# teofum/platinum

Hardware: AMD Instinct MI355X
Metric: Msamples/s (paths x spp x bounces / s) at 1920x1080, 8 bounces (higher is better)
Workload: dtype f32; 1 GPU; C3 1.04M-triangle instanced sphere field, 1920x1080; width=1920, height=1080, max_bounces=8, samples_in_flight=128, spp_per_gpu=1792, spp_total=1792, integrator=MIS+NEE, flags=MultiscatterGGX, triangles=1036300, call_pattern=render(spp_per_step) per step, batches=14, nonfinite_policy=zero (a NaN/inf sample counts as black; parity default is propagate), parallelism=sample-sharded x1, one process per GPU + RCCL all-reduce

## Files before the change

include/ptamd.h:

```cpp
#ifndef PTAMD_H
#define PTAMD_H

#include <stdint.h>

#ifdef __cplusplus
extern "C" {
#endif

#define PT_ABI_VERSION 5u


enum { PT_STATUS_BLOCKED = 0, PT_STATUS_READY = 1, PT_STATUS_BUSY = 4, PT_STATUS_DONE = 8 };
enum { PT_INTEGRATOR_SIMPLE = 0, PT_INTEGRATOR_MIS = 1 };
enum { PT_FLAG_NONE = 0, PT_FLAG_MULTISCATTER_GGX = 1 << 0, PT_FLAG_GMON = 1 << 1 };
enum { PT_NONFINITE_PROPAGATE = 0, PT_NONFINITE_ZERO = 1 };
enum {
  PT_MATERIAL_THIN_DIELECTRIC = 1 << 0,
  PT_MATERIAL_USE_ALPHA = 1 << 1,
  PT_MATERIAL_EMISSIVE = 1 << 2,
  PT_MATERIAL_ANISOTROPIC = 1 << 3
};

typedef enum pt_error {
  PT_OK = 0,
// ... 219 lines not shown
  float agx_offset[3], agx_slope[3], agx_power[3], agx_saturation;
  float khr_compression_start, khr_desaturation;
  float flim_pre_exposure, flim_pre_formation_filter[3], flim_pre_formation_filter_strength;
  float flim_extended_gamut_scale[3], flim_extended_gamut_rotation[3], flim_extended_gamut_mul[3];
  float flim_sigmoid_log2_min, flim_sigmoid_log2_max, flim_sigmoid_toe[2], flim_sigmoid_shoulder[2];
  float flim_negative_exposure, flim_negative_density, flim_print_backlight[3], flim_print_exposure, flim_print_density;
  float flim_black_point;
  uint32_t flim_auto_black_point;
  float flim_post_formation_filter[3], flim_post_formation_filter_strength, flim_midtone_saturation;
  float shadow_color[3], midtone_color[3], highlight_color[3];
  float shadow_offset, midtone_offset, highlight_offset;
  pt_colorspace output_space;
} pt_tonemap_options;

void pt_default_post_options(pt_post_options* o);
void pt_default_tonemap_options(pt_tonemap_options* o);
int pt_set_post_options(pt_renderer* r, const pt_post_options* o);
int pt_set_tonemap_options(pt_renderer* r, const pt_tonemap_options* o);
int pt_read_render_target(pt_renderer* r, uint8_t* rgba8_out);
int pt_present_render_target(pt_renderer* r, void** device_rgba8_out, void** stream_out);

int pt_read_accumulator(pt_renderer* r, float* rgba_out);
void* pt_accumulator_device_ptr(pt_renderer* r);


typedef struct pt_denoise_options {
  uint32_t enabled;
  uint32_t iterations;
  float sigma_luminance, sigma_normal, sigma_depth;
  uint32_t apply_to_target;
} pt_denoise_options;
enum { PT_AOV_ALBEDO = 0, PT_AOV_NORMAL = 1, PT_AOV_MOMENTS = 2 };
void pt_default_denoise_options(pt_denoise_options* o);
int pt_set_denoise_options(pt_renderer* r, const pt_denoise_options* o);
int pt_read_aov(pt_renderer* r, uint32_t aov, float* rgba_out);
int pt_read_denoised(pt_renderer* r, float* rgba_out);

typedef struct pt_despeckle_options {
  uint32_t enabled;
  float threshold;
} pt_despeckle_options;
void pt_default_despeckle_options(pt_despeckle_options* o);
int pt_set_despeckle_options(pt_renderer* r, const pt_despeckle_options* o);

typedef struct pt_exposure_options {
  uint32_t enabled;
  float target_log2;
  float low_fraction;
  float high_fraction;
  float min_ev, max_ev;
  float smoothing;
} pt_exposure_options;
void pt_default_exposure_options(pt_exposure_options* o);
int pt_set_exposure_options(pt_renderer* r, const pt_exposure_options* o);
int pt_reset_exposure(pt_renderer* r);

typedef struct pt_exposure_meter {
  uint32_t bins[256];
  uint32_t below, above, nonfinite, metered;
  uint32_t kept;  uint32_t _pad;  uint64_t weighted;
  float mean_log2, target_ev, ev, gain;
} pt_exposure_meter;
int pt_read_exposure_meter(pt_renderer* r, pt_exposure_meter* out);
int pt_debug_exposure(pt_renderer* r, const float* rgba, uint32_t width, uint32_t height, const uint32_t* rect,
                      const pt_exposure_options* options, pt_exposure_meter* out, float* scaled_out);

typedef struct pt_adaptive_options {
  uint32_t enabled;
  float threshold;
  uint32_t min_spp;
  uint32_t interval;
} pt_adaptive_options;
void pt_default_adaptive_options(pt_adaptive_options* o);
int pt_set_adaptive_options(pt_renderer* r, const pt_adaptive_options* o);
int pt_read_sample_counts(pt_renderer* r, uint32_t* out);

typedef struct pt_render_region {
  uint32_t enabled;
  uint32_t x0, y0, x1, y1;
} pt_render_region;
void pt_default_render_region(pt_render_region* o);
int pt_set_render_region(pt_renderer* r, const pt_render_region* o);
int pt_region_tiles(uint32_t width, uint32_t height, const pt_render_region* o, uint32_t* tiles_out, uint32_t capacity, uint32_t* count);

const char* pt_last_error(void);


int pt_get_constants(const pt_renderer* r, pt_constants* out);
int pt_get_env_alias(const pt_renderer* r, pt_alias_entry* out, uint64_t capacity, uint64_t* count);
int pt_get_lights(const pt_renderer* r, pt_area_light* out, uint32_t capacity, uint32_t* count);

typedef struct pt_hit_record {
  float t, u, v;
  int32_t instance;
  int32_t primitive;
} pt_hit_record;
int pt_trace_primary(pt_renderer* r, uint32_t sample_idx, pt_hit_record* out );

int pt_debug_sample(pt_renderer* r, uint32_t sample_idx, float* radiance_out, int32_t* hits_out);

typedef struct pt_stats {
  uint64_t triangles;
  uint64_t bvh_nodes;
  uint32_t bvh_max_depth;
  uint32_t samples_in_flight;
  double upload_ms;
  double bvh_build_ms;
  uint64_t closest_rays;
  uint64_t shadow_rays;
  uint64_t shaded_hits;
  uint64_t paths;
  uint64_t nonfinite_samples;
  double ms_raygen, ms_closest, ms_shade, ms_shadow, ms_accumulate;
  uint64_t launches_closest, launches_shadow;
  double nodes_per_closest_ray, tris_per_closest_ray;
  double nodes_per_shadow_ray, tris_per_shadow_ray;
  uint32_t accel_two_level;
  uint32_t batches;
  uint64_t leaf_slots;
} pt_stats;
int pt_get_stats(pt_renderer* r, pt_stats* out);
int pt_set_profiling(pt_renderer* r, int enabled);
int pt_measure_traversal(pt_renderer* r, uint32_t sample_idx);

#ifdef __cplusplus
}
#endif
#endif
```

platinum_amd/abi.py:

```python
import ctypes as C
import os

PT_ABI_VERSION = 5

STATUS_BLOCKED, STATUS_READY, STATUS_BUSY, STATUS_DONE = 0, 1, 4, 8
INTEGRATOR_SIMPLE, INTEGRATOR_MIS = 0, 1
FLAG_NONE, FLAG_MULTISCATTER_GGX, FLAG_GMON = 0, 1, 2
MATERIAL_THIN_DIELECTRIC, MATERIAL_USE_ALPHA, MATERIAL_EMISSIVE, MATERIAL_ANISOTROPIC = 1, 2, 4, 8
NONFINITE_PROPAGATE, NONFINITE_ZERO = 0, 1
ACCEL_AUTO, ACCEL_ONE_BVH, ACCEL_TWO_LEVEL = 0, 1, 2


class Float3(C.Structure):
    _fields_ = [("x", C.c_float), ("y", C.c_float), ("z", C.c_float), ("_pad", C.c_float)]


class VertexData(C.Structure):
    _fields_ = [("normal", Float3), ("tangent", C.c_float * 4), ("texCoords", C.c_float * 2), ("_pad", C.c_float * 2)]


class MaterialGPU(C.Structure):
    _fields_ = [
        ("baseColor", C.c_float * 4), ("emission", Float3), ("emissionStrength", C.c_float),
        ("roughness", C.c_float), ("metallic", C.c_float), ("transmission", C.c_float), ("ior", C.c_float),
# ... 81 lines not shown


class CreateInfo(C.Structure):
    _fields_ = [
        ("abi_version", C.c_uint32), ("device_ordinal", C.c_int32), ("lut_blob", C.c_void_p),
        ("lut_blob_size", C.c_uint64), ("lut_path", C.c_char_p),
        ("device_ordinals", C.POINTER(C.c_int32)), ("device_count", C.c_uint32),
    ]


class RenderParams(C.Structure):
    _fields_ = [
        ("width", C.c_uint32), ("height", C.c_uint32), ("spp", C.c_uint32), ("gmon_buckets", C.c_uint32),
        ("flags", C.c_int32), ("integrator", C.c_uint32), ("working_space", Colorspace),
        ("max_bounces", C.c_uint32), ("first_sample", C.c_uint32), ("samples_in_flight", C.c_uint32),
        ("nonfinite_policy", C.c_uint32), ("external_accumulator", C.c_void_p), ("stream", C.c_void_p),
        ("accel_structure", C.c_uint32), ("_reserved", C.c_uint32),
    ]


class QueuePlan(C.Structure):
    _fields_ = [("samples_in_flight", C.c_uint32), ("tiles_per_seg", C.c_uint32), ("nseg", C.c_uint32), ("seg_cap", C.c_uint32),
                ("capacity", C.c_uint64), ("lbuf_entries", C.c_uint64)]


class GmonOptions(C.Structure):
    _fields_ = [("cap", C.c_float)]


class PostOptions(C.Structure):
    _fields_ = [(n, C.c_float) for n in (
        "exposure", "ca_amount", "ca_green_shift", "contrast", "saturation", "blacks", "shadows", "highlights", "whites",
        "vig_amount", "vig_midpoint", "vig_feather", "vig_power", "vig_roundness")]


class TonemapOptions(C.Structure):
    _fields_ = [
        ("tonemapper", C.c_uint32), ("agx_offset", C.c_float * 3), ("agx_slope", C.c_float * 3), ("agx_power", C.c_float * 3),
        ("agx_saturation", C.c_float), ("khr_compression_start", C.c_float), ("khr_desaturation", C.c_float),
        ("flim_pre_exposure", C.c_float), ("flim_pre_formation_filter", C.c_float * 3), ("flim_pre_formation_filter_strength", C.c_float),
        ("flim_extended_gamut_scale", C.c_float * 3), ("flim_extended_gamut_rotation", C.c_float * 3), ("flim_extended_gamut_mul", C.c_float * 3),
        ("flim_sigmoid_log2_min", C.c_float), ("flim_sigmoid_log2_max", C.c_float), ("flim_sigmoid_toe", C.c_float * 2),
        ("flim_sigmoid_shoulder", C.c_float * 2), ("flim_negative_exposure", C.c_float), ("flim_negative_density", C.c_float),
        ("flim_print_backlight", C.c_float * 3), ("flim_print_exposure", C.c_float), ("flim_print_density", C.c_float),
        ("flim_black_point", C.c_float), ("flim_auto_black_point", C.c_uint32), ("flim_post_formation_filter", C.c_float * 3),
        ("flim_post_formation_filter_strength", C.c_float), ("flim_midtone_saturation", C.c_float),
        ("shadow_color", C.c_float * 3), ("midtone_color", C.c_float * 3), ("highlight_color", C.c_float * 3),
        ("shadow_offset", C.c_float), ("midtone_offset", C.c_float), ("highlight_offset", C.c_float), ("output_space", Colorspace),
    ]


TONEMAP_NONE, TONEMAP_AGX, TONEMAP_KHRONOS_PBR, TONEMAP_FLIM = 0, 1, 2, 3


class DenoiseOptions(C.Structure):
    _fields_ = [("enabled", C.c_uint32), ("iterations", C.c_uint32), ("sigma_luminance", C.c_float), ("sigma_normal", C.c_float),
                ("sigma_depth", C.c_float), ("apply_to_target", C.c_uint32)]


AOV_ALBEDO, AOV_NORMAL, AOV_MOMENTS = 0, 1, 2


class DespeckleOptions(C.Structure):
    _fields_ = [("enabled", C.c_uint32), ("threshold", C.c_float)]


class ExposureOptions(C.Structure):
    _fields_ = [("enabled", C.c_uint32), ("target_log2", C.c_float), ("low_fraction", C.c_float), ("high_fraction", C.c_float),
                ("min_ev", C.c_float), ("max_ev", C.c_float), ("smoothing", C.c_float)]


class ExposureMeter(C.Structure):
    _fields_ = [("bins", C.c_uint32 * 256), ("below", C.c_uint32), ("above", C.c_uint32), ("nonfinite", C.c_uint32), ("metered", C.c_uint32),
                ("kept", C.c_uint32), ("_pad", C.c_uint32), ("weighted", C.c_uint64),
                ("mean_log2", C.c_float), ("target_ev", C.c_float), ("ev", C.c_float), ("gain", C.c_float)]


class AdaptiveOptions(C.Structure):
    _fields_ = [("enabled", C.c_uint32), ("threshold", C.c_float), ("min_spp", C.c_uint32), ("interval", C.c_uint32)]


class RenderRegion(C.Structure):
    _fields_ = [("enabled", C.c_uint32), ("x0", C.c_uint32), ("y0", C.c_uint32), ("x1", C.c_uint32), ("y1", C.c_uint32)]


class HitRecord(C.Structure):
    _fields_ = [("t", C.c_float), ("u", C.c_float), ("v", C.c_float), ("instance", C.c_int32), ("primitive", C.c_int32)]


class Stats(C.Structure):
    _fields_ = [
        ("triangles", C.c_uint64), ("bvh_nodes", C.c_uint64), ("bvh_max_depth", C.c_uint32),
        ("samples_in_flight", C.c_uint32), ("upload_ms", C.c_double), ("bvh_build_ms", C.c_double),
        ("closest_rays", C.c_uint64), ("shadow_rays", C.c_uint64), ("shaded_hits", C.c_uint64), ("paths", C.c_uint64),
        ("nonfinite_samples", C.c_uint64), ("ms_raygen", C.c_double), ("ms_closest", C.c_double), ("ms_shade", C.c_double), ("ms_shadow", C.c_double),
        ("ms_accumulate", C.c_double), ("launches_closest", C.c_uint64), ("launches_shadow", C.c_uint64),
        ("nodes_per_closest_ray", C.c_double), ("tris_per_closest_ray", C.c_double),
        ("nodes_per_shadow_ray", C.c_double), ("tris_per_shadow_ray", C.c_double),
        ("accel_two_level", C.c_uint32), ("batches", C.c_uint32), ("leaf_slots", C.c_uint64),
    ]


class RuntimeInfo(C.Structure):
    _fields_ = [
        ("hip_runtime_path", C.c_char * 512), ("hsa_runtime_path", C.c_char * 512), ("rccl_path", C.c_char * 512),
        ("hip_runtimes_mapped", C.c_uint32), ("hsa_runtimes_mapped", C.c_uint32), ("rccl_mapped", C.c_uint32),
        ("hip_runtime_version", C.c_int32), ("all_mapped", C.c_char * 2048),
    ]


assert C.sizeof(Float3) == 16 and C.sizeof(VertexData) == 48 and C.sizeof(MaterialGPU) == 96
assert C.sizeof(Instance) == 64 and C.sizeof(CameraData) == 80 and C.sizeof(Constants) == 176
assert C.sizeof(AreaLight) == 48

SYMBOLS = [
    ("pt_create", C.c_int, [C.POINTER(CreateInfo), C.POINTER(C.c_void_p)]),
    ("pt_group_partition", C.c_int, [C.c_uint32, C.c_uint32, C.c_int32, C.c_uint32, C.POINTER(C.c_uint64), C.POINTER(C.c_uint64),
                                     C.POINTER(C.c_uint32), C.POINTER(C.c_uint32)]),
    ("pt_get_runtime_info", C.c_int, [C.POINTER(RuntimeInfo)]),
    ("pt_rccl_probe", C.c_int, []),
    ("pt_rccl_selftest", C.c_int, [C.c_int32]),
    ("pt_plan_queues", C.c_int, [C.c_uint32, C.c_uint32, C.c_uint32, C.c_uint32, C.c_uint64, C.c_uint32, C.c_uint32, C.POINTER(QueuePlan)]),
    ("pt_destroy", None, [C.c_void_p]),
    ("pt_start_render", C.c_int, [C.c_void_p, C.POINTER(SceneSnapshot), C.POINTER(RenderParams)]),
    ("pt_render_step", C.c_int, [C.c_void_p, C.c_uint32]),
    ("pt_wait", C.c_int, [C.c_void_p]),
    ("pt_status", C.c_int, [C.c_void_p]),
    ("pt_progress", C.c_int, [C.c_void_p, C.POINTER(C.c_uint64), C.POINTER(C.c_uint64)]),
    ("pt_render_time_ms", C.c_uint64, [C.c_void_p]),
    ("pt_read_accumulator", C.c_int, [C.c_void_p, C.c_void_p]),
    ("pt_accumulator_device_ptr", C.c_void_p, [C.c_void_p]),
    ("pt_set_gmon_options", C.c_int, [C.c_void_p, C.POINTER(GmonOptions)]),
    ("pt_default_post_options", None, [C.POINTER(PostOptions)]),
    ("pt_default_tonemap_options", None, [C.POINTER(TonemapOptions)]),
    ("pt_set_post_options", C.c_int, [C.c_void_p, C.POINTER(PostOptions)]),
    ("pt_set_tonemap_options", C.c_int, [C.c_void_p, C.POINTER(TonemapOptions)]),
    ("pt_read_render_target", C.c_int, [C.c_void_p, C.c_void_p]),
    ("pt_present_render_target", C.c_int, [C.c_void_p, C.POINTER(C.c_void_p), C.POINTER(C.c_void_p)]),
    ("pt_read_gmon_bucket", C.c_int, [C.c_void_p, C.c_uint32, C.c_void_p]),
    ("pt_default_denoise_options", None, [C.POINTER(DenoiseOptions)]),
    ("pt_set_denoise_options", C.c_int, [C.c_void_p, C.POINTER(DenoiseOptions)]),
    ("pt_read_aov", C.c_int, [C.c_void_p, C.c_uint32, C.c_void_p]),
    ("pt_read_denoised", C.c_int, [C.c_void_p, C.c_void_p]),
    ("pt_default_despeckle_options", None, [C.POINTER(DespeckleOptions)]),
    ("pt_set_despeckle_options", C.c_int, [C.c_void_p, C.POINTER(DespeckleOptions)]),
    ("pt_default_exposure_options", None, [C.POINTER(ExposureOptions)]),
    ("pt_set_exposure_options", C.c_int, [C.c_void_p, C.POINTER(ExposureOptions)]),
    ("pt_reset_exposure", C.c_int, [C.c_void_p]),
    ("pt_read_exposure_meter", C.c_int, [C.c_void_p, C.POINTER(ExposureMeter)]),
    ("pt_debug_exposure", C.c_int, [C.c_void_p, C.c_void_p, C.c_uint32, C.c_uint32, C.c_void_p, C.POINTER(ExposureOptions),
                                    C.POINTER(ExposureMeter), C.c_void_p]),
    ("pt_default_adaptive_options", None, [C.POINTER(AdaptiveOptions)]),
    ("pt_set_adaptive_options", C.c_int, [C.c_void_p, C.POINTER(AdaptiveOptions)]),
    ("pt_read_sample_counts", C.c_int, [C.c_void_p, C.c_void_p]),
    ("pt_default_render_region", None, [C.POINTER(RenderRegion)]),
    ("pt_set_render_region", C.c_int, [C.c_void_p, C.POINTER(RenderRegion)]),
    ("pt_region_tiles", C.c_int, [C.c_uint32, C.c_uint32, C.POINTER(RenderRegion), C.c_void_p, C.c_uint32, C.POINTER(C.c_uint32)]),
    ("pt_last_error", C.c_char_p, []),
    ("pt_get_constants", C.c_int, [C.c_void_p, C.POINTER(Constants)]),
    ("pt_get_lights", C.c_int, [C.c_void_p, C.c_void_p, C.c_uint32, C.POINTER(C.c_uint32)]),
    ("pt_get_env_alias", C.c_int, [C.c_void_p, C.c_void_p, C.c_uint64, C.POINTER(C.c_uint64)]),
    ("pt_trace_primary", C.c_int, [C.c_void_p, C.c_uint32, C.c_void_p]),
    ("pt_debug_sample", C.c_int, [C.c_void_p, C.c_uint32, C.c_void_p, C.c_void_p]),
    ("pt_get_stats", C.c_int, [C.c_void_p, C.POINTER(Stats)]),
    ("pt_set_profiling", C.c_int, [C.c_void_p, C.c_int]),
    ("pt_measure_traversal", C.c_int, [C.c_void_p, C.c_uint32]),
]

_PKG_DIR = os.path.dirname(os.path.abspath(__file__))
LIB_PATH = os.path.join(_PKG_DIR, "csrc", "libptamd.so")
LUT_PATH = os.path.join(_PKG_DIR, "data", "ggx_luts.bin")

_lib = None


class PtamdError(RuntimeError):
    pass


def library_path():
    return os.environ.get("PTAMD_LIB", LIB_PATH)


def _mapped_objects(prefix):
    found = []
    try:
        with open("/proc/self/maps") as f:
            for line in f:
                parts = line.split(None, 5)
                if len(parts) == 6 and os.path.basename(parts[5].strip()).startswith(prefix) and parts[5].strip() not in found:
                    found.append(parts[5].strip())
    except OSError:
        pass
    return found


def _torch_bundled_hip():
    import importlib.util
    try:
        spec = importlib.util.find_spec("torch")
    except (ImportError, ValueError):
        return None
    if spec is None or not spec.submodule_search_locations:
        return None
    import glob
    for d in spec.submodule_search_locations:
        p = os.path.join(d, "lib", "libamdhip64.so")
        if os.path.exists(p):
            return p
        versioned = sorted(glob.glob(p + ".*"))
        if versioned:
            return versioned[0]
    return None


def _elf_dynamic_strings(path, tag):
    import struct
    try:
        with open(path, "rb") as f:
            hdr = f.read(0x40)
            if hdr[:4] != b"\x7fELF" or hdr[4] != 2 or hdr[5] != 1:
                return []
            shoff, = struct.unpack_from("<Q", hdr, 0x28)
            shentsize, shnum = struct.unpack_from("<HH", hdr, 0x3A)
            if shentsize < 64 or shnum == 0 or shnum > 4096:
                return []
            f.seek(shoff)
            sh = f.read(shentsize * shnum)
            secs = [struct.unpack_from("<IIQQQQIIQQ", sh, i * shentsize) for i in range(shnum)]
            out = []
            for sec in secs:
                if sec[1] != 6:
                    continue
                strsec = secs[sec[6]]
                f.seek(sec[4]); dyn = f.read(sec[5])
                f.seek(strsec[4]); strtab = f.read(strsec[5])
                for off in range(0, len(dyn) - 15, 16):
                    t, v = struct.unpack_from("<qQ", dyn, off)
                    if t == 0:
                        break
# ... 74 lines not shown
```

platinum_amd/csrc/kernels.h:

```cpp
#pragma once
#include <hip/hip_runtime.h>

#include "pt_device.h"
#include "pt_layout.h"
#include "pt_post.h"

namespace pt {

constexpr int kBlock = 256;

struct WaveStats { unsigned long long closest, shadow, shaded, paths; };

struct Segments {
  uint32_t* active[2];
  uint32_t* shadow;
  uint32_t* poison;
  WaveStats* stats;
  uint32_t* table_closest;
  uint32_t* table_shadow;
  uint32_t* shade_order;
  uint32_t* shade_cost;
  uint32_t seg_cap;
  uint32_t nseg;
  uint32_t tiles_per_seg;
  uint32_t nsamples;
  uint32_t bands;
  uint32_t nstats;
  uint32_t refill_threshold;
};
PT_HD uint32_t segment_first_tile(const Segments& seg, uint32_t sg) { return segment_first_tile(seg.nseg, seg.bands, seg.tiles_per_seg, sg); }
PT_HD uint32_t segment_lbuf_base(const Segments& seg, uint32_t sg) { return segment_lbuf_base(seg.nseg, seg.bands, seg.tiles_per_seg, seg.nsamples, sg); }
__device__ __forceinline__ uint32_t wave_lane() { return __builtin_amdgcn_mbcnt_hi(~0u, __builtin_amdgcn_mbcnt_lo(~0u, 0u)); }

void launch_raygen(hipStream_t s, uint32_t grid, const DeviceScene& S, PathState st, vec4* Lbuf, Segments seg, BatchCounters* ctr,
                   uint32_t first_sample, uint32_t nsamples);
void launch_raygen_adaptive(hipStream_t s, uint32_t grid, const DeviceScene& S, PathState st, vec4* Lbuf, Segments seg,
                            uint32_t first_sample, uint32_t nsamples, const Rect& rect, const uint32_t* active, const uint32_t* active_count);
void launch_chunk_tables(hipStream_t s, Segments seg, uint32_t cur, BatchCounters* ctr, uint32_t bounce_closest,
                         uint32_t bounce_shadow, bool do_shadow);
uint32_t trace_block_threads(bool two_level);
uint32_t trace_blocks_per_cu_two_level();
void launch_trace_closest(hipStream_t s, uint32_t grid, const DeviceScene& S, PathState st, vec4* hit, Segments seg, uint32_t cur,
                          BatchCounters* ctr, uint32_t bounce, uint32_t* spill, int32_t* hitlog, uint32_t log_stride, bool count);
uint32_t shade_block_threads();
uint32_t shade_blocks_per_cu();
void launch_shade(hipStream_t s, uint32_t grid, const DeviceScene* S_device, PathState sin, PathState sout, const vec4* hit,
                  ShadowQueue sq, vec4* Lbuf, Segments seg, uint32_t cur, BatchCounters* ctr, uint32_t bounce);
void launch_trace_shadow(hipStream_t s, uint32_t grid, const DeviceScene& S, ShadowQueue sq, vec4* Lbuf, Segments seg,
                         BatchCounters* ctr, uint32_t bounce, uint32_t* spill, bool count);
void launch_accumulate(hipStream_t s, vec4* acc, const vec4* Lbuf, uint32_t npixels, uint32_t width, uint32_t nsamples, uint32_t n0,
                       uint32_t nonfinite_policy, BatchCounters* ctr);
void launch_accumulate_adaptive(hipStream_t s, vec4* acc, const vec4* Lbuf, uint32_t npixels, uint32_t width, uint32_t nsamples, uint32_t n0,
                                uint32_t nonfinite_policy, BatchCounters* ctr, const uint32_t* active, const uint32_t* active_count,
                                uint32_t max_active, vec2* mom, uint32_t* tile_n, const Rect& rect);
void launch_accumulate_gmon(hipStream_t s, vec4* buckets, const vec4* Lbuf, uint32_t npixels, uint32_t width, uint32_t nsamples, uint32_t n0,
                            uint32_t samples_per_bucket, uint32_t gmon_buckets, uint32_t bucket_base, uint32_t nonfinite_policy, BatchCounters* ctr);
void launch_weighted_add(hipStream_t s, vec4* out, const vec4* in, float w, uint32_t npixels, bool first, bool last);
void launch_gmon(hipStream_t s, vec4* acc, const vec4* buckets, uint32_t npixels, uint32_t nBuckets, float cap);
void launch_postprocess(hipStream_t s, const vec4* acc, uint32_t* rgba8, uint32_t W, uint32_t H, const PostConstants& pc);
void launch_fold_counters(hipStream_t s, const BatchCounters* ctr, Totals* tot, Segments seg, bool counted);
void launch_shade_records(hipStream_t s, const DeviceScene& S, ShadeRec* out);
void launch_light_records(hipStream_t s, const DeviceScene& S, LightRec* out, float* cdf);
void launch_hit_records(hipStream_t s, uint32_t grid, const DeviceScene& S, PathState st, const vec4* hit, Segments seg,
                        pt_hit_record* out);

struct LbvhResult {
  BvhNode* nodes = nullptr;
  TriRec* tris = nullptr;
  uint32_t slot_count = 0;
  MeshTrav* mesh_trav = nullptr;
  uint32_t root_ref = kInvalidRef;
  uint32_t node_count = 0;
  uint32_t max_depth = 0;
  uint32_t depth4 = 0;
  bool wide6 = false;
};
struct LbvhScratch {
  char* base = nullptr;
  size_t cap = 0;
  hipError_t ensure(size_t bytes);
  void release();
};
struct PrimTables { const uint32_t* prim_tri = nullptr; const uint32_t* mesh_prim_base = nullptr; const uint32_t* inst_prim_base = nullptr; uint32_t slot_count = 0; };
hipError_t build_lbvh(hipStream_t s, const DeviceScene& S, const PrimTables& prims, uint32_t instance_count, uint32_t stack_capacity,
                      LbvhScratch* scratch, LbvhResult* out);
hipError_t build_two_level(hipStream_t s, const DeviceScene& S, const MeshInfo* meshes, uint32_t mesh_count, uint32_t instance_count,
                           uint32_t tri_count, uint32_t stack_capacity, LbvhScratch* scratch, LbvhResult* out);

}
```

platinum_amd/csrc/kernels.hip:

```cpp
#include <hip/hip_runtime.h>

#include "kernels.h"
#include "pt_denoise.h"
#include "pt_post.h"
#include "pt_shade.h"
#include "queue_plan.h"

namespace pt {

__device__ __forceinline__ vec4 ld_stream(const vec4* p) {
  using f4 = __attribute__((ext_vector_type(4))) float;
  const f4 v = __builtin_nontemporal_load((const f4*)p);
  return vec4{v.x, v.y, v.z, v.w};
}
__device__ __forceinline__ uint32_t ld_stream(const uint32_t* p) { return __builtin_nontemporal_load(p); }
__device__ __forceinline__ void st_stream(vec4* p, vec4 v) {
  using f4 = __attribute__((ext_vector_type(4))) float;
  __builtin_nontemporal_store(f4{v.x, v.y, v.z, v.w}, (f4*)p);
}
__device__ __forceinline__ void st_stream(uint32_t* p, uint32_t v) { __builtin_nontemporal_store(v, p); }

__device__ __forceinline__ uint32_t wave_prefix(unsigned long long mask) {
  return __builtin_amdgcn_mbcnt_hi((uint32_t)(mask >> 32), __builtin_amdgcn_mbcnt_lo((uint32_t)mask, 0u));
}
__device__ __forceinline__ uint32_t wave_sum(uint32_t v) {
  for (int off = 32; off > 0; off >>= 1) v += __shfl_xor(v, off, 64);
  return v;
}
__device__ __forceinline__ uint32_t wave_index() { return blockIdx.x * (blockDim.x >> 6) + (threadIdx.x >> 6); }
__device__ __forceinline__ uint32_t wave_count() { return gridDim.x * (blockDim.x >> 6); }
#ifdef PT_TAIL_PROBE
#define PT_TAIL_BEGIN const unsigned long long tail_t0 = wall_clock64(); unsigned long long tail_take = 0, tail_setup = 0, tail_ta = 0;
#define PT_TAIL_T(acc) { const unsigned long long tb_ = wall_clock64(); acc += tb_ - tail_ta; tail_ta = tb_; }
#define PT_TAIL_MARK tail_ta = wall_clock64();
#define PT_TAIL_END(kind)                                                                                         \
  if (wave_lane() == 0 && bounce < 16u) {                                                                           \
    const unsigned long long t1 = wall_clock64();                                                                   \
    atomicMax(&ctr->tail_end_max[kind][bounce], t1); atomicAdd(&ctr->tail_end_sum[kind][bounce], t1);              \
    atomicMax(&ctr->tail_start_inv[kind][bounce], ~tail_t0); atomicAdd(&ctr->tail_waves[kind][bounce], 1ull);     \
    atomicAdd(&ctr->tail_take[kind][bounce], tail_take); atomicAdd(&ctr->tail_setup[kind][bounce], tail_setup);     \
    atomicAdd(&ctr->tail_busy[kind][bounce], t1 - tail_t0);                                                         \
  }
#else
#define PT_TAIL_BEGIN
#define PT_TAIL_END(kind)
#define PT_TAIL_T(acc)
#define PT_TAIL_MARK
#endif

constexpr uint32_t kClaimMax = 8;

__device__ __forceinline__ uint32_t chunk_entry(uint32_t sg, uint32_t k, uint32_t rays) { return ((rays - 1u) << 26) | (k << 16) | sg; }
static_assert(kMaxSegments <= 65536 && kMaxSegmentSlots / 64 <= 1024, "chunk_entry packs 16 + 10 + 6 bits");

struct ChunkClaims {
  const uint32_t* __restrict__ table;
  uint32_t* cursor;
  uint32_t nseg, total, lane;
  uint32_t next_c, end_c, run_c = 0;
  uint32_t e0 = 0, e1 = 0, e2 = 0, e3 = 0, e4 = 0, e5 = 0, e6 = 0, e7 = 0;
  uint32_t claim_k = kClaimMax, nwaves_grid = 1;
  __device__ __forceinline__ void init(const uint32_t* tab, uint32_t total_, uint32_t* cur, const Segments& seg, uint32_t lane_) {
    table = tab; total = total_; cursor = cur; nseg = seg.nseg; lane = lane_;
    next_c = end_c = 0;
    nwaves_grid = gridDim.x * (blockDim.x >> 6);
    claim_k = guided(total);
  }
  __device__ __forceinline__ uint32_t guided(uint32_t remaining) const {
    return remaining > 32u * nwaves_grid ? kClaimMax : remaining > 8u * nwaves_grid ? 4u : remaining > 2u * nwaves_grid ? 2u : 1u;
  }
  uint32_t pool_next = 0, pool_end = 0;
  bool exhausted = false;
  __device__ __forceinline__ uint32_t take(bool need) {
    uint32_t got = kInvalidRef;
    for (;;) {
      const unsigned long long m = __ballot(need && got == kInvalidRef);
      if (m == 0) return got;
      if (pool_next == pool_end) {
        if (exhausted) return got;
        if (next_c == end_c) {
          uint32_t base = 0;
          if (lane == 0) base = atomicAdd(cursor, claim_k);
          base = __builtin_amdgcn_readfirstlane(base);
          if (base >= total) { exhausted = true; return got; }
          next_c = run_c = base;
// ... 145 lines not shown
    const uint32_t first_tile = segment_first_tile(seg, sg);
    for (uint32_t k = 0; k < seg.tiles_per_seg * nsamples; k++) {
      const uint32_t tile = first_tile + k / nsamples;
      if (tile >= tiles) break;
      const uint32_t r = (k % nsamples) * 64u + lane;
      const uint32_t pl = r / nsamples, s = r - pl * nsamples;
      const PixelXY q = tile_pixel(active[tile], pl, tilesX);
      const bool valid = rect_contains(rect, q.x, q.y);
      RayGenOut rg;
      if (valid) rg = stage_raygen(S, q.x, q.y, first_sample + s);
      const unsigned long long m = __ballot(valid);
      if (valid) {
        const uint32_t j = seg_slot(seg.nseg, sg, n_out + wave_prefix(m));
        const uint32_t pid = lbuf_index(tile, s, nsamples, pl);
        const uint32_t rel = pid - first_tile * nsamples * 64u;
        st.rayO[j] = vec4{rg.o.x, rg.o.y, rg.o.z, 0.0f};
        st.rayD[j] = vec4{rg.d.x, rg.d.y, rg.d.z, u2f((rg.dim & kMetaDimMask) | (rel << kMetaPidShift))};
        st.att[j] = vec4{1.0f, 1.0f, 1.0f, u2f(rg.offset)};
        Lbuf[pid] = vec4{0.0f, 0.0f, 0.0f, 1.0f};
      }
      n_out += (uint32_t)__popcll(m);
    }
    if (lane == 0) { seg.active[0][sg] = n_out; seg.poison[sg] = 0u; }
    started += n_out;
  }
  if (lane == 0) {
    WaveStats& ws = seg.stats[wave_index()];
    ws.paths += started;
    ws.closest += started;
  }
}

#ifndef PT_TWO_BLOCK
#define PT_TWO_BLOCK 1024
#define PT_TWO_BLOCKS_PER_CU 1
#define PT_TWO_LDS_NODES 1024
#endif
constexpr uint32_t kTraceBlock2 = PT_TWO_BLOCK;
constexpr uint32_t kLdsNodes = PT_TWO_LDS_NODES;
#ifndef PT_TRI_VOTE
#define PT_TRI_VOTE 2
#endif
template <bool ANY, bool COUNT, bool TWO, bool W6 = false>
__device__ __forceinline__ void wave_traverse(const DeviceScene& S, const BvhNode* lds_nodes, TravState& ts, TraversalCount* tc) {
  constexpr int kRoom = W6 ? 1 : 4, kRows = W6 ? kPendLeaves6 : kPendLeaves;
  if (ts.cur != kInvalidRef && ts.st.npend <= kRows - kRoom) {
    if (TWO) {
      trav_leave(ts);
      const bool at_inst = ts.cur != kInvalidRef && (ts.cur & kInstBit) != 0;
      const bool at_node = ts.cur != kInvalidRef && !at_inst;
      const unsigned long long mi = __ballot(at_inst), mn = __ballot(at_node);
      if (mi != 0 && (2 * __popcll(mi) >= __popcll(mn) || mn == 0)) {
        if (at_inst) trav_resolve(S, ts);
      } else if (at_node) {
        if (lds_nodes) trav_node<COUNT, true>(lds_nodes, ts, tc); else trav_node<COUNT, true>(S.nodes, ts, tc);
      }
    } else if (W6) {
      trav_node6<COUNT>(S.nodes, ts, tc);
    } else {
      trav_node<COUNT, false>(S.nodes, ts, tc);
    }
  }
  const bool pending = ts.st.npend > 0;
  const bool stuck = pending && (ts.cur == kInvalidRef || ts.st.npend > kRows - kRoom);
  const bool advancing = ts.cur != kInvalidRef && !stuck;
  const unsigned long long mp = __ballot(pending);
  if (mp == 0) return;
  const bool go = PT_TRI_VOTE * __popcll(mp) >= __popcll(__ballot(1)) || __ballot(ts.st.npend > kRows - kRoom) != 0 || __ballot(advancing) == 0;
  if (go && pending) {
    const bool fin = W6 ? trav_pending_leaf6<ANY, COUNT>(S, ts, tc) : trav_pending_leaf<ANY, COUNT>(S, ts, tc);
    if (fin) { ts.cur = kInvalidRef; ts.st.npend = 0; ts.st.sp = 0; }
  }
}

__device__ __forceinline__ const BvhNode* stage_nodes(const DeviceScene& S, BvhNode* lds_nodes) {
  if (S.node_count > kLdsNodes) return nullptr;
  const uint4* src = reinterpret_cast<const uint4*>(S.nodes);
  uint4* dst = reinterpret_cast<uint4*>(lds_nodes);
  for (uint32_t i = threadIdx.x; i < S.node_count * 4; i += blockDim.x) dst[i] = src[i];
  __syncthreads();
  return lds_nodes;
}

template <bool COUNT, bool TWO, bool W6 = false>
__global__ void __launch_bounds__(TWO ? kTraceBlock2 : kBlock, TWO ? PT_TWO_BLOCKS_PER_CU : PT_CLOSEST_WAVES)
k_trace_closest(DeviceScene S, PathState st, vec4* __restrict__ hit, Segments seg, uint32_t cur, BatchCounters* __restrict__ ctr, uint32_t bounce,
                uint32_t* __restrict__ spill, int32_t* __restrict__ hitlog, uint32_t log_stride) {
  PT_TAIL_BEGIN
  constexpr uint32_t kTB = TWO ? kTraceBlock2 : kBlock;
  __shared__ uint32_t lds_stack[(W6 ? kLdsStack6 : kLdsStack) + 1][kTB];
  __shared__ uint32_t lds_pend[(W6 ? kPendLeaves6 : kPendLeaves) + 1][kTB];
  __shared__ BvhNode lds_nodes_buf[TWO && kLdsNodes ? kLdsNodes : 1];
  const BvhNode* lds_nodes = TWO && kLdsNodes ? stage_nodes(S, lds_nodes_buf) : nullptr;
  const uint32_t lane = wave_lane();
  ChunkClaims src;
  src.init(seg.table_closest, ctr->chunks_closest[bounce], &ctr->work_closest[bounce], seg, lane);
  TraversalStack stack;
  stack.lds = &lds_stack[0][threadIdx.x];
  stack.pend = &lds_pend[0][threadIdx.x];
  stack.lds_stride = kTB;
  stack.spill = spill + ((size_t)blockIdx.x * kTB + threadIdx.x);
  stack.spill_stride = gridDim.x * kTB;
  TraversalCount tc;

  TravState ts;
  uint32_t ray = kInvalidRef;
  auto finish = [&]() {
    const RayHit& h = ts.best;
#ifdef PT_DEBUG_PID
    if (ts.dbg) printf("dbg finish: t %.9g u %.9g v %.9g tri %u gid %u\n", h.t, h.u, h.v, h.tri, h.gid >> 2);
    ts.dbg = false;
#endif
    hit[ray] = vec4{h.t, h.u, h.v, u2f(h.tri == kInvalidRef ? kInvalidRef : (h.tri | ((h.gid & 3u) << 28)))};
    if (hitlog) {
      const uint32_t pixel = pixel_of_pid_1spp(segment_lbuf_base(seg, slot_segment(seg.nseg, ray)) + (f2u(st.rayD[ray].w) >> kMetaPidShift), S.width);
      int32_t* hl = &hitlog[((size_t)bounce * log_stride + pixel) * 2];
      hl[0] = hl[1] = -1;
      if (h.tri != kInvalidRef) triangle_ids(S, h.tri, &hl[0], &hl[1]);
    }
    ray = kInvalidRef;
  };
  const uint32_t refill = seg.refill_threshold;
  for (;;) {
    PT_TAIL_MARK
    const uint32_t fresh = src.take(ray == kInvalidRef);
    PT_TAIL_T(tail_take)
    if (fresh != kInvalidRef) {
      ray = fresh;
      const vec4 o4 = st.rayO[ray];
      const vec4 d4 = st.rayD[ray];
      float ir = 0.0f;
      if (S.has_alpha) ir = Halton{halton_table(S.halton), f2u(st.att[ray].w), f2u(d4.w) & kMetaDimMask}.sample1d();
#ifdef PT_DEBUG_PID
      ts.dbg = ctr->_pad[1] == bounce + 1u && segment_lbuf_base(seg, slot_segment(seg.nseg, ray)) + (f2u(d4.w) >> kMetaPidShift) == ctr->_pad[0];
      if (ts.dbg) printf("dbg ray slot %u lane %u wave %u o %.9g %.9g %.9g d %.9g %.9g %.9g\n", ray, lane, wave_index(), o4.x, o4.y, o4.z, d4.x, d4.y, d4.z);
#endif
      if (trav_init(S, ts, v3(o4.x, o4.y, o4.z), v3(d4.x, d4.y, d4.z), 1e-3f, kInf, ir, stack, false, COUNT ? &tc : nullptr)) finish();
    }
    PT_TAIL_T(tail_setup)
    if (__ballot(ray != kInvalidRef) == 0) {
      if (src.exhausted && src.pool_next == src.pool_end) break;
      continue;
    }
    while (ray != kInvalidRef) {
      wave_traverse<false, COUNT, TWO, W6>(S, lds_nodes, ts, &tc);
      if (ts.cur == kInvalidRef && ts.st.npend == 0) finish();
      if (refill && !src.exhausted && (uint32_t)__popcll(__ballot(ray != kInvalidRef)) < refill) break;
    }
  }
  if (COUNT) {
    const uint32_t nn = wave_sum(tc.nodes), t = wave_sum(tc.tris);
    if (lane == 0) {
      atomicAdd(&ctr->nodes_closest, (unsigned long long)nn);
      atomicAdd(&ctr->tris_closest, (unsigned long long)t);
    }
  }
  PT_TAIL_END(0)
}

#ifndef PT_SHADE_WAVES
#define PT_SHADE_WAVES 4
#endif
#ifndef PT_SHADE_BLOCK
#define PT_SHADE_BLOCK 256
#endif
constexpr uint32_t kShadeBlock = PT_SHADE_BLOCK;
constexpr uint32_t kShadeHalton = 128;
constexpr uint32_t kShadeLights = 64;
constexpr int kLutE = 128, kLutEavg = 128, kLutEavgMs = 32;
constexpr uint32_t kBinCap = 128;

__global__ void __launch_bounds__(PT_SHADE_BLOCK, (PT_SHADE_WAVES * 4 * 64) / PT_SHADE_BLOCK)
k_shade(const DeviceScene* __restrict__ Sp, PathState sin, PathState sout, const vec4* __restrict__ hit, ShadowQueue sq,
        vec4* __restrict__ Lbuf, Segments seg, uint32_t cur, BatchCounters* __restrict__ ctr, uint32_t bounce) {
  PT_TAIL_BEGIN
  const DeviceScene& S = *Sp;
  __shared__ HaltonEntry lds_halton[kShadeHalton];
  __shared__ LightRec lds_lights[kShadeLights];
  __shared__ float lds_Eavg[kLutEavg];
  __shared__ float lds_EavgMs[kLutEavgMs * kLutEavgMs];
  static_assert(kMaxSegmentSlots <= 65536, "slot numbers inside a segment are binned as uint16_t (queue_plan.h bounds seg_cap)");
  __shared__ uint16_t lds_bins[kShadeBlock / 64][5][kBinCap];
  __shared__ uint32_t lds_bin_tri[kShadeBlock / 64][5][kBinCap];
  const uint32_t halton_base = 5u + 7u * bounce;
  uint32_t halton_count = 11u + 5u * bounce;
  if (halton_base >= (uint32_t)kHaltonDims) halton_count = 0;
  else if (halton_base + halton_count > (uint32_t)kHaltonDims) halton_count = (uint32_t)kHaltonDims - halton_base;
  if (halton_count > kShadeHalton) halton_count = kShadeHalton;
  const bool lights_in_lds = S.lightCount <= kShadeLights;
  {
    const uint4* src = reinterpret_cast<const uint4*>(S.halton + halton_base);
    uint4* dst = reinterpret_cast<uint4*>(lds_halton);
    for (uint32_t i = threadIdx.x; i < halton_count * 2; i += kShadeBlock) dst[i] = ldg(&src[i]);
    if (lights_in_lds) {
      const uint4* ls = reinterpret_cast<const uint4*>(S.light_recs);
      uint4* ld = reinterpret_cast<uint4*>(lds_lights);
      for (uint32_t i = threadIdx.x; i < S.lightCount * (uint32_t)(sizeof(LightRec) / 16); i += kShadeBlock) ld[i] = ldg(&ls[i]);
    }
    for (uint32_t i = threadIdx.x; i < (uint32_t)kLutEavg; i += kShadeBlock) lds_Eavg[i] = ldg(&S.luts.Eavg.d[i]);
    for (uint32_t i = threadIdx.x; i < (uint32_t)(kLutEavgMs * kLutEavgMs); i += kShadeBlock) lds_EavgMs[i] = ldg(&S.luts.EavgMs.d[i]);
  }
  __syncthreads();
  ShadeTables T;
  T.luts.E = Lut{S.luts.E.d, kLutE, kLutE, 1, 0};
  T.luts.Eavg = Lut{lds_Eavg, kLutEavg, 1, 1, 1};
  T.luts.EMs = Lut{S.luts.EMs.d, S.luts.EMs.w, S.luts.EMs.h, S.luts.EMs.depth, 0};
  T.luts.EavgMs = Lut{lds_EavgMs, kLutEavgMs, kLutEavgMs, 1, 1};
  T.luts.ETransIn = Lut{S.luts.ETransIn.d, S.luts.ETransIn.w, S.luts.ETransIn.h, S.luts.ETransIn.depth, 0};
  T.luts.ETransOut = Lut{S.luts.ETransOut.d, S.luts.ETransOut.w, S.luts.ETransOut.h, S.luts.ETransOut.depth, 0};
  T.halton = HaltonTab{S.halton, lds_halton, halton_base, halton_count};
  T.lights = lights_in_lds ? lds_lights : S.light_recs;
  T.light_cdf = S.light_cdf;
  T.lights_lds = lights_in_lds ? 1 : 0;

  const uint32_t lane = wave_lane();
  uint32_t shaded = 0, total_out = 0, total_shadow = 0;
  uint32_t claim = wave_index();
  uint16_t* bin = &lds_bins[threadIdx.x >> 6][0][0];
  uint32_t* bin_tri = &lds_bin_tri[threadIdx.x >> 6][0][0];
  while (claim < seg.nseg) {
    const uint32_t sg = __builtin_amdgcn_readfirstlane(seg.shade_order[claim]);
    const unsigned long long seg_t0 = wall_clock64();
    const uint32_t lbuf_base = segment_lbuf_base(seg, sg);
    const uint32_t n = __builtin_amdgcn_readfirstlane(seg.active[cur][sg]);
    uint32_t n_out = 0, n_shadow = 0;
    const uint32_t seg_poisoned = S.env_texture < 0 ? __builtin_amdgcn_readfirstlane(seg.poison[sg]) : 0u;
    unsigned long long poisoned_now = 0;
    uint32_t cnt0 = 0, cnt1 = 0, cnt2 = 0, cnt3 = 0, cnt4 = 0;
    uint32_t k0 = 0;
    for (;;) {
      while (k0 < n && cnt0 < 64 && cnt1 < 64 && cnt2 < 64 && cnt3 < 64 && cnt4 < 64) {
        const uint32_t k = k0 + lane;
        uint32_t cls = 5;
        uint32_t w = 0;
        if (k < n) {
          w = f2u(hit[seg_slot(seg.nseg, sg, k)].w);
          cls = w == kInvalidRef ? 4u : (w >> 28) & 3u;
          if (w == kInvalidRef && S.env_texture < 0) {
            if (!seg_poisoned) cls = 5u;
            else {
// ... 377 lines not shown
    tot->shadow_rays += t[1];
    tot->shaded_hits += t[2];
    tot->paths += t[3];
    tot->nonfinite += ctr->nonfinite;
  } else {
    tot->nodes_closest += ctr->nodes_closest; tot->tris_closest += ctr->tris_closest;
    tot->nodes_shadow += ctr->nodes_shadow; tot->tris_shadow += ctr->tris_shadow;
    tot->counted_closest += t[0]; tot->counted_shadow += t[1];
  }
}

__global__ void __launch_bounds__(kBlock) k_light_records(DeviceScene S, LightRec* __restrict__ out, float* __restrict__ cdf) {
  const uint32_t i = blockIdx.x * kBlock + threadIdx.x;
  if (i < S.lightCount) { out[i] = make_light_rec(S, S.lights[i]); cdf[i] = S.lights[i].cumulativePower; }
}

__global__ void __launch_bounds__(kBlock) k_shade_records(DeviceScene S, ShadeRec* __restrict__ out) {
  const uint32_t t = blockIdx.x * kBlock + threadIdx.x;
  if (t >= 2u * S.slot_count) return;
  const TriRec& tr = S.tris[t >> 1];
  const uint32_t gid = (t & 1u) ? tr.gid_b : tr.gid_a;
  if (gid == kInvalidRef) { out[t] = ShadeRec{}; return; }
  const uint32_t inst = tr.inst_code & kSlotInstMask;
  out[t] = make_shade_rec(S, inst, (gid >> 2) - S.instances[inst].tri_global_base);
}

__global__ void __launch_bounds__(kBlock) k_hit_records(DeviceScene S, PathState st, const vec4* __restrict__ hit, Segments seg,
                                                         pt_hit_record* __restrict__ out) {
  const uint32_t lane = wave_lane();
  for (uint32_t sg = wave_index(); sg < seg.nseg; sg += wave_count()) {
    const uint32_t n = seg.active[0][sg];
    for (uint32_t k = lane; k < n; k += 64) {
      const uint32_t i = seg_slot(seg.nseg, sg, k);
      const vec4 h = hit[i];
      const uint32_t tri = f2u(h.w) == kInvalidRef ? kInvalidRef : (f2u(h.w) & kHitTriMask);
      pt_hit_record r;
      if (tri != kInvalidRef) {
        r.t = h.x; r.u = h.y; r.v = h.z;
        triangle_ids(S, tri, &r.instance, &r.primitive);
      } else {
        r.t = 0.0f; r.u = 0.0f; r.v = 0.0f; r.instance = -1; r.primitive = -1;
      }
      out[pixel_of_pid_1spp(segment_lbuf_base(seg, sg) + (f2u(st.rayD[i].w) >> kMetaPidShift), S.width)] = r;
    }
  }
}

void launch_raygen(hipStream_t s, uint32_t grid, const DeviceScene& S, PathState st, vec4* Lbuf, Segments seg, BatchCounters* ctr,
                   uint32_t first_sample, uint32_t nsamples) {
  hipLaunchKernelGGL(k_raygen, dim3(grid), dim3(kBlock), 0, s, S, st, Lbuf, seg, ctr, first_sample, nsamples, tiles_x(S.width), tiles_y(S.height));
}
void launch_raygen_adaptive(hipStream_t s, uint32_t grid, const DeviceScene& S, PathState st, vec4* Lbuf, Segments seg,
                            uint32_t first_sample, uint32_t nsamples, const Rect& rect, const uint32_t* active, const uint32_t* active_count) {
  hipLaunchKernelGGL(k_raygen_adaptive, dim3(grid), dim3(kBlock), 0, s, S, st, Lbuf, seg, first_sample, nsamples, tiles_x(S.width), rect, active,
                     active_count);
}
void launch_chunk_tables(hipStream_t s, Segments seg, uint32_t cur, BatchCounters* ctr, uint32_t bounce_closest,
                         uint32_t bounce_shadow, bool do_shadow) {
  hipLaunchKernelGGL(k_chunk_tables, dim3(kTableBlocks, 3), dim3(1024), 0, s, seg, cur, ctr, bounce_closest, bounce_shadow, do_shadow ? 1u : 0u);
}
uint32_t trace_block_threads(bool two_level) { return two_level ? kTraceBlock2 : (uint32_t)kBlock; }
uint32_t trace_blocks_per_cu_two_level() { return PT_TWO_BLOCKS_PER_CU; }
void launch_trace_closest(hipStream_t s, uint32_t grid, const DeviceScene& S, PathState st, vec4* hit, Segments seg, uint32_t cur,
                          BatchCounters* ctr, uint32_t bounce, uint32_t* spill, int32_t* hitlog, uint32_t log_stride, bool count) {
  if (S.two_level) {
    if (count)
      hipLaunchKernelGGL((k_trace_closest<true, true>), dim3(grid), dim3(kTraceBlock2), 0, s, S, st, hit, seg, cur, ctr, bounce, spill, hitlog, log_stride);
    else
      hipLaunchKernelGGL((k_trace_closest<false, true>), dim3(grid), dim3(kTraceBlock2), 0, s, S, st, hit, seg, cur, ctr, bounce, spill, hitlog, log_stride);
    return;
  }
  if (S.wide6) {
    if (count)
      hipLaunchKernelGGL((k_trace_closest<true, false, true>), dim3(grid), dim3(kBlock), 0, s, S, st, hit, seg, cur, ctr, bounce, spill, hitlog, log_stride);
    else
      hipLaunchKernelGGL((k_trace_closest<false, false, true>), dim3(grid), dim3(kBlock), 0, s, S, st, hit, seg, cur, ctr, bounce, spill, hitlog, log_stride);
    return;
  }
  if (count)
    hipLaunchKernelGGL((k_trace_closest<true, false>), dim3(grid), dim3(kBlock), 0, s, S, st, hit, seg, cur, ctr, bounce, spill, hitlog, log_stride);
  else
    hipLaunchKernelGGL((k_trace_closest<false, false>), dim3(grid), dim3(kBlock), 0, s, S, st, hit, seg, cur, ctr, bounce, spill, hitlog, log_stride);
}
uint32_t shade_block_threads() { return kShadeBlock; }
uint32_t shade_blocks_per_cu() { return (PT_SHADE_WAVES * 4 * 64) / PT_SHADE_BLOCK; }
void launch_shade(hipStream_t s, uint32_t grid, const DeviceScene* S, PathState sin, PathState sout, const vec4* hit,
                  ShadowQueue sq, vec4* Lbuf, Segments seg, uint32_t cur, BatchCounters* ctr, uint32_t bounce) {
  hipLaunchKernelGGL(k_shade, dim3(grid), dim3(kShadeBlock), 0, s, S, sin, sout, hit, sq, Lbuf, seg, cur, ctr, bounce);
}
void launch_trace_shadow(hipStream_t s, uint32_t grid, const DeviceScene& S, ShadowQueue sq, vec4* Lbuf, Segments seg,
                         BatchCounters* ctr, uint32_t bounce, uint32_t* spill, bool count) {
  if (S.two_level) {
    if (count) hipLaunchKernelGGL((k_trace_shadow<true, true>), dim3(grid), dim3(kTraceBlock2), 0, s, S, sq, Lbuf, seg, ctr, bounce, spill);
    else hipLaunchKernelGGL((k_trace_shadow<false, true>), dim3(grid), dim3(kTraceBlock2), 0, s, S, sq, Lbuf, seg, ctr, bounce, spill);
    return;
  }
  if (S.wide6) {
    if (count) hipLaunchKernelGGL((k_trace_shadow<true, false, true>), dim3(grid), dim3(kBlock), 0, s, S, sq, Lbuf, seg, ctr, bounce, spill);
    else hipLaunchKernelGGL((k_trace_shadow<false, false, true>), dim3(grid), dim3(kBlock), 0, s, S, sq, Lbuf, seg, ctr, bounce, spill);
    return;
  }
  if (count) hipLaunchKernelGGL((k_trace_shadow<true, false>), dim3(grid), dim3(kBlock), 0, s, S, sq, Lbuf, seg, ctr, bounce, spill);
  else hipLaunchKernelGGL((k_trace_shadow<false, false>), dim3(grid), dim3(kBlock), 0, s, S, sq, Lbuf, seg, ctr, bounce, spill);
}
void launch_accumulate(hipStream_t s, vec4* acc, const vec4* Lbuf, uint32_t npixels, uint32_t width, uint32_t nsamples, uint32_t n0,
                       uint32_t nonfinite_policy, BatchCounters* ctr) {
  const uint32_t tiles = tile_count(width, npixels / width);
  hipLaunchKernelGGL(k_accumulate, dim3((tiles + kBlock / 64 - 1) / (kBlock / 64)), dim3(kBlock), 0, s, acc, Lbuf, npixels, width, nsamples, n0,
                     nonfinite_policy, ctr);
}
void launch_accumulate_adaptive(hipStream_t s, vec4* acc, const vec4* Lbuf, uint32_t npixels, uint32_t width, uint32_t nsamples, uint32_t n0,
                                uint32_t nonfinite_policy, BatchCounters* ctr, const uint32_t* active, const uint32_t* active_count,
                                uint32_t max_active, vec2* mom, uint32_t* tile_n, const Rect& rect) {
  const uint32_t tiles = max_active;
  hipLaunchKernelGGL(k_accumulate_adaptive, dim3((tiles + kBlock / 64 - 1) / (kBlock / 64)), dim3(kBlock), 0, s, acc, Lbuf, npixels, width, nsamples,
                     n0, nonfinite_policy, ctr, active, active_count, mom, tile_n, rect);
}
void launch_accumulate_gmon(hipStream_t s, vec4* buckets, const vec4* Lbuf, uint32_t npixels, uint32_t width, uint32_t nsamples, uint32_t n0,
                            uint32_t samples_per_bucket, uint32_t gmon_buckets, uint32_t bucket_base, uint32_t nonfinite_policy, BatchCounters* ctr) {
  hipLaunchKernelGGL(k_accumulate_gmon, dim3((npixels + kBlock - 1) / kBlock), dim3(kBlock), 0, s, buckets, Lbuf, npixels, width, nsamples, n0,
                     samples_per_bucket, gmon_buckets, bucket_base, nonfinite_policy, ctr);
}
void launch_weighted_add(hipStream_t s, vec4* out, const vec4* in, float w, uint32_t npixels, bool first, bool last) {
  hipLaunchKernelGGL(k_weighted_add, dim3((npixels + kBlock - 1) / kBlock), dim3(kBlock), 0, s, out, in, w, npixels, first ? 1u : 0u, last ? 1u : 0u);
}
void launch_gmon(hipStream_t s, vec4* acc, const vec4* buckets, uint32_t npixels, uint32_t nBuckets, float cap) {
  hipLaunchKernelGGL(k_gmon, dim3((npixels + kBlock - 1) / kBlock), dim3(kBlock), 0, s, acc, buckets, npixels, nBuckets, cap);
}
void launch_postprocess(hipStream_t s, const vec4* acc, uint32_t* rgba8, uint32_t W, uint32_t H, const PostConstants& pc) {
  hipLaunchKernelGGL(k_postprocess, dim3((W * H + kBlock - 1) / kBlock), dim3(kBlock), 0, s, acc, rgba8, W, H, pc);
}
void launch_fold_counters(hipStream_t s, const BatchCounters* ctr, Totals* tot, Segments seg, bool counted) {
  hipLaunchKernelGGL(k_fold_counters, dim3(1), dim3(kBlock), 0, s, ctr, tot, seg, counted ? 1u : 0u);
}
void launch_shade_records(hipStream_t s, const DeviceScene& S, ShadeRec* out) {
  if (S.slot_count) hipLaunchKernelGGL(k_shade_records, dim3((2u * S.slot_count + kBlock - 1) / kBlock), dim3(kBlock), 0, s, S, out);
}
void launch_light_records(hipStream_t s, const DeviceScene& S, LightRec* out, float* cdf) {
  if (S.lightCount) hipLaunchKernelGGL(k_light_records, dim3((S.lightCount + kBlock - 1) / kBlock), dim3(kBlock), 0, s, S, out, cdf);
}
void launch_hit_records(hipStream_t s, uint32_t grid, const DeviceScene& S, PathState st, const vec4* hit, Segments seg,
                        pt_hit_record* out) {
  hipLaunchKernelGGL(k_hit_records, dim3(grid), dim3(kBlock), 0, s, S, st, hit, seg, out);
}

}
```

platinum_amd/csrc/multi_device.hip:

```cpp
#include <dlfcn.h>
#include <rccl/rccl.h>

#include <algorithm>
#include <condition_variable>
#include <functional>
#include <mutex>
#include <thread>

#include "renderer_state.h"
#include "runtime_identity.h"

namespace {

struct Worker {
  std::mutex m;
  std::condition_variable cv;
  std::function<int()> job;
  bool has = false, stop = false;
  int rc = PT_OK;
  std::string err;
  std::thread th;
  Worker() { th = std::thread([this] { run(); }); }
  ~Worker() {
    { std::lock_guard<std::mutex> l(m); stop = true; }
// ... 620 lines not shown
int pt_measure_traversal(pt_renderer* r, uint32_t sample_idx) {
  if (!is_group(r)) return dev_measure_traversal(r, sample_idx);
  pt_renderer* m = first_started(r->group);
  return m ? dev_measure_traversal(m, sample_idx) : fail(PT_ERR_BAD_STATE, "no render started");
}

int pt_set_profiling(pt_renderer* r, int enabled) {
  if (!is_group(r)) return dev_set_profiling(r, enabled);
  for (auto* m : r->group->shards) { int rc = dev_set_profiling(m, enabled); if (rc != PT_OK) return rc; }
  return PT_OK;
}

int pt_set_denoise_options(pt_renderer* r, const pt_denoise_options* o) {
  if (!is_group(r)) return dev_set_denoise_options(r, o);
  if (!o) return fail(PT_ERR_INVALID_ARGUMENT, "null argument");
  if (o->enabled) return fail(PT_ERR_UNSUPPORTED, "pt_set_denoise_options: a device group does not keep AOVs");
  for (auto* m : r->group->shards) { int rc = dev_set_denoise_options(m, o); if (rc != PT_OK) return rc; }
  return PT_OK;
}

int pt_set_despeckle_options(pt_renderer* r, const pt_despeckle_options* o) {
  if (!is_group(r)) return dev_set_despeckle_options(r, o);
  if (!o) return fail(PT_ERR_INVALID_ARGUMENT, "null argument");
  if (o->enabled) return fail(PT_ERR_UNSUPPORTED, "pt_set_despeckle_options: a device group does not run the denoiser");
  for (auto* m : r->group->shards) { int rc = dev_set_despeckle_options(m, o); if (rc != PT_OK) return rc; }
  return PT_OK;
}

int pt_read_aov(pt_renderer* r, uint32_t aov, float* rgba_out) {
  if (!is_group(r)) return dev_read_aov(r, aov, rgba_out);
  return fail(PT_ERR_BAD_STATE, "pt_read_aov: a device group does not keep AOVs");
}

int pt_read_denoised(pt_renderer* r, float* rgba_out) {
  if (!is_group(r)) return dev_read_denoised(r, rgba_out);
  return fail(PT_ERR_BAD_STATE, "pt_read_denoised: a device group does not keep AOVs");
}

int pt_set_exposure_options(pt_renderer* r, const pt_exposure_options* o) {
  if (!is_group(r)) return dev_set_exposure_options(r, o);
  for (auto* m : r->group->shards) { int rc = dev_set_exposure_options(m, o); if (rc != PT_OK) return rc; }
  return PT_OK;
}

int pt_reset_exposure(pt_renderer* r) {
  if (!is_group(r)) return dev_reset_exposure(r);
  for (auto* m : r->group->shards) { int rc = dev_reset_exposure(m); if (rc != PT_OK) return rc; }
  return PT_OK;
}

int pt_read_exposure_meter(pt_renderer* r, pt_exposure_meter* out) {
  if (!is_group(r)) return dev_read_exposure_meter(r, nullptr, out);
  if (!out) return fail(PT_ERR_INVALID_ARGUMENT, "null argument");
  DeviceGroup* grp = r->group;
  if (!grp->started) return fail(PT_ERR_BAD_STATE, "pt_read_exposure_meter before pt_start_render");
  int rc = group_wait(r);
  if (rc != PT_OK) return rc;
  pt_renderer* m = first_started(grp);
  if (!m || m->device != grp->shards[0]->device) return fail(PT_ERR_BAD_STATE, "device group: no member on the first device has samples");
  return dev_read_exposure_meter(m, grp->merged, out);
}

int pt_debug_exposure(pt_renderer* r, const float* rgba, uint32_t width, uint32_t height, const uint32_t* rect, const pt_exposure_options* options,
                      pt_exposure_meter* out, float* scaled_out) {
  return dev_debug_exposure(is_group(r) ? r->group->shards[0] : r, rgba, width, height, rect, options, out, scaled_out);
}

int pt_set_adaptive_options(pt_renderer* r, const pt_adaptive_options* o) {
  if (!is_group(r)) return dev_set_adaptive_options(r, o);
  if (!o) return fail(PT_ERR_INVALID_ARGUMENT, "null argument");
  if (o->enabled) return fail(PT_ERR_UNSUPPORTED, "pt_set_adaptive_options: a device group does not sample adaptively");
  for (auto* m : r->group->shards) { int rc = dev_set_adaptive_options(m, o); if (rc != PT_OK) return rc; }
  return PT_OK;
}

int pt_set_render_region(pt_renderer* r, const pt_render_region* o) {
  if (!is_group(r)) return dev_set_render_region(r, o);
  if (!o) return fail(PT_ERR_INVALID_ARGUMENT, "null argument");
  if (o->enabled) return fail(PT_ERR_UNSUPPORTED, "pt_set_render_region: a device group does not render regions");
  for (auto* m : r->group->shards) { int rc = dev_set_render_region(m, o); if (rc != PT_OK) return rc; }
  return PT_OK;
}

int pt_read_sample_counts(pt_renderer* r, uint32_t* out) {
  if (!is_group(r)) return dev_read_sample_counts(r, out);
  if (!out) return fail(PT_ERR_INVALID_ARGUMENT, "null argument");
  DeviceGroup* grp = r->group;
  if (!grp->started) return fail(PT_ERR_BAD_STATE, "pt_read_sample_counts before pt_start_render");
  int rc = group_wait(r);
  if (rc != PT_OK) return rc;
  uint64_t n = 0;
  for (auto* m : grp->shards) if (m->started) n += m->launched;
  std::fill(out, out + (size_t)grp->params.width * grp->params.height, (uint32_t)n);
  return PT_OK;
}

int pt_get_stats(pt_renderer* r, pt_stats* out) {
  if (!r || !out) return fail(PT_ERR_INVALID_ARGUMENT, "null argument");
  return is_group(r) ? group_get_stats(r, out) : dev_get_stats(r, out);
}

}
```

platinum_amd/csrc/pt_bvh.h:

```cpp
#pragma once
#include "pt_bsdf.h"

namespace pt {

struct RayHit {
  float t, u, v;
  uint32_t tri;
  uint32_t gid;
};

PT_HD bool intersect_triangle(vec3 o, vec3 d, float tmin, float tmax, vec3 v0, vec3 e1, vec3 e2, float* t_out, float* u_out,
                              float* v_out) {
  const vec3 p = cross(d, e2);
  const float det = dot(e1, p);
  if (!(fabsf(det) > (1e-6f * ((fabsf(e1.x) + fabsf(e1.y)) + fabsf(e1.z))) * ((fabsf(p.x) + fabsf(p.y)) + fabsf(p.z)))) return false;
  const float inv = 1.0f / det;
  const vec3 s = o - v0;
  const float u = dot(s, p) * inv;
  if (!(u >= 0.0f && u <= 1.0f)) return false;
  const vec3 q = cross(s, e1);
  const float v = dot(d, q) * inv;
  if (!(v >= 0.0f && u + v <= 1.0f)) return false;
  const float t = dot(e2, q) * inv;
  if (!(t >= tmin && t <= tmax)) return false;
// ... 271 lines not shown
  const BvhNode n = nodes[ts.cur];
  if (COUNT) cnt->nodes++;
  const vec3 ro = TWO ? ts.co : ts.o, ri = TWO ? ts.cinv : ts.inv;
  const bool gx = TWO ? ts.cnegx : ts.negx, gy = TWO ? ts.cnegy : ts.negy, gz = TWO ? ts.cnegz : ts.negz;
  const float ax = node_scale(n.exp[0]) * ri.x, ay = node_scale(n.exp[1]) * ri.y, az = node_scale(n.exp[2]) * ri.z;
  const float bx = (n.origin[0] - ro.x) * ri.x, by = (n.origin[1] - ro.y) * ri.y, bz = (n.origin[2] - ro.z) * ri.z;
  const float bnx = TWO ? bx - ts.sx : bx, bny = TWO ? by - ts.sy : by, bnz = TWO ? bz - ts.sz : bz;
  const float bfx = TWO ? bx + ts.sx : bx, bfy = TWO ? by + ts.sy : by, bfz = TWO ? bz + ts.sz : bz;
  const uint32_t nx = gx ? n.qhi[0] : n.qlo[0], fx = gx ? n.qlo[0] : n.qhi[0];
  const uint32_t ny = gy ? n.qhi[1] : n.qlo[1], fy = gy ? n.qlo[1] : n.qhi[1];
  const uint32_t nz = gz ? n.qhi[2] : n.qlo[2], fz = gz ? n.qlo[2] : n.qhi[2];
  const float far_lim = ts.best.t * kCullSlack;
  float dist[4];
#pragma unroll
  for (int k = 0; k < 4; k++) {
    const float tnx = __builtin_fmaf((float)((nx >> (8 * k)) & 0xffu), ax, bnx), tfx = __builtin_fmaf((float)((fx >> (8 * k)) & 0xffu), ax, bfx);
    const float tny = __builtin_fmaf((float)((ny >> (8 * k)) & 0xffu), ay, bny), tfy = __builtin_fmaf((float)((fy >> (8 * k)) & 0xffu), ay, bfy);
    const float tnz = __builtin_fmaf((float)((nz >> (8 * k)) & 0xffu), az, bnz), tfz = __builtin_fmaf((float)((fz >> (8 * k)) & 0xffu), az, bfz);
    const float tn = fmaxf(fmaxf(fmaxf(tnx, tny), tnz), ts.tmin);
    const float tf = fminf(fminf(fminf(tfx, tfy), tfz), far_lim);
    const bool hit = n.ref[k] != kInvalidRef && tn <= __builtin_fmaf(tf, kSlabSlack, 1e-30f);
    const bool leaf = hit && (n.ref[k] & kLeafBit);
    dist[k] = hit && !leaf ? tn : kInf;
    ts.st.pend[(leaf ? ts.st.npend : kPendLeaves) * ts.st.lds_stride] = TWO ? n.ref[k] + ts.tri_base : n.ref[k];
    ts.st.npend += leaf ? 1 : 0;
  }
  float d0 = dist[0], d1 = dist[1], d2 = dist[2], d3 = dist[3];
  uint32_t r0 = n.ref[0], r1 = n.ref[1], r2 = n.ref[2], r3 = n.ref[3];
#define PT_CSWAP(da, ra, db, rb) { const bool sw = db < da; const float td = sw ? db : da; const uint32_t tr = sw ? rb : ra; \
                                   db = sw ? da : db; rb = sw ? ra : rb; da = td; ra = tr; }
  PT_CSWAP(d0, r0, d1, r1) PT_CSWAP(d2, r2, d3, r3) PT_CSWAP(d0, r0, d2, r2) PT_CSWAP(d1, r1, d3, r3) PT_CSWAP(d1, r1, d2, r2)
#undef PT_CSWAP
  if (d0 < kInf) {
    if (d3 < kInf) ts.st.push(r3);
    if (d2 < kInf) ts.st.push(r2);
    if (d1 < kInf) ts.st.push(r1);
    ts.cur = r0;
  } else {
    ts.cur = ts.st.sp == 0 ? kInvalidRef : ts.st.pop();
  }
}

PT_HD BvhNode6 quantize_node6(const Box3* boxes, int n_int, int n_leaf, uint32_t base_node, uint32_t base_leaf) {
  BvhNode6 n;
  const int count = n_int + n_leaf;
  float lo[3] = {kInf, kInf, kInf}, hi[3] = {-kInf, -kInf, -kInf};
  for (int k = 0; k < count; k++)
    for (int a = 0; a < 3; a++) {
      lo[a] = fminf(lo[a], boxes[k].lo[a]);
      hi[a] = fmaxf(hi[a], boxes[k].hi[a]);
    }
  n.counts = (uint8_t)(n_int | (n_leaf << 3));
  n.base_node = base_node;
  n.base_leaf = base_leaf;
  n._pad = 0;
  for (int a = 0; a < 3; a++) {
    n.origin[a] = lo[a];
    const float need = (hi[a] - lo[a]) * (1.0f / 255.0f);
    uint32_t e = (f2u(need) >> 23) & 0xffu;
    if ((f2u(need) & 0x7fffffu) != 0) e += 1;
    if (e < 1) e = 1;
    if (e > 254) e = 254;
    while (e < 254 && lo[a] + 255.0f * node_scale((uint8_t)e) < hi[a]) e += 1;
    n.exp[a] = (uint8_t)e;
    const float scale = node_scale((uint8_t)e), inv = 1.0f / scale;
    uint32_t qlo[6], qhi[6];
    for (int k = 0; k < 6; k++) {
      if (k >= count) { qlo[k] = 255u; qhi[k] = 0u; continue; }
      int ql = (int)floorf((boxes[k].lo[a] - lo[a]) * inv);
      ql = ql < 0 ? 0 : (ql > 255 ? 255 : ql);
      while (ql > 0 && lo[a] + (float)ql * scale > boxes[k].lo[a]) ql--;
      int qh = (int)ceilf((boxes[k].hi[a] - lo[a]) * inv);
      qh = qh < 0 ? 0 : (qh > 255 ? 255 : qh);
      while (qh < 255 && lo[a] + (float)qh * scale < boxes[k].hi[a]) qh++;
      qlo[k] = (uint32_t)ql; qhi[k] = (uint32_t)qh;
    }
    n.q[a][0] = qlo[0] | qlo[1] << 8 | qlo[2] << 16 | qlo[3] << 24;
    n.q[a][1] = qhi[0] | qhi[1] << 8 | qhi[2] << 16 | qhi[3] << 24;
    n.q[a][2] = qlo[4] | qlo[5] << 8 | qhi[4] << 16 | qhi[5] << 24;
  }
  return n;
}

template <bool COUNT>
PT_HD void trav_node6(const BvhNode* __restrict__ nodes, TravState& ts, TraversalCount* cnt) {
  const BvhNode6 n = reinterpret_cast<const BvhNode6*>(nodes)[ts.cur];
  if (COUNT) cnt->nodes++;
  const float ax = node_scale(n.exp[0]) * ts.inv.x, ay = node_scale(n.exp[1]) * ts.inv.y, az = node_scale(n.exp[2]) * ts.inv.z;
  const float bx = (n.origin[0] - ts.o.x) * ts.inv.x, by = (n.origin[1] - ts.o.y) * ts.inv.y, bz = (n.origin[2] - ts.o.z) * ts.inv.z;
  const uint32_t nx = ts.negx ? n.q[0][1] : n.q[0][0], fx = ts.negx ? n.q[0][0] : n.q[0][1];
  const uint32_t ny = ts.negy ? n.q[1][1] : n.q[1][0], fy = ts.negy ? n.q[1][0] : n.q[1][1];
  const uint32_t nz = ts.negz ? n.q[2][1] : n.q[2][0], fz = ts.negz ? n.q[2][0] : n.q[2][1];
  const uint32_t nx2 = ts.negx ? n.q[0][2] >> 16 : n.q[0][2], fx2 = ts.negx ? n.q[0][2] : n.q[0][2] >> 16;
  const uint32_t ny2 = ts.negy ? n.q[1][2] >> 16 : n.q[1][2], fy2 = ts.negy ? n.q[1][2] : n.q[1][2] >> 16;
  const uint32_t nz2 = ts.negz ? n.q[2][2] >> 16 : n.q[2][2], fz2 = ts.negz ? n.q[2][2] : n.q[2][2] >> 16;
  const uint32_t n_int = n.counts & 7u, count = n_int + ((n.counts >> 3) & 7u);
  const float far_lim = ts.best.t * kCullSlack;
  float best_d = kInf;
  uint32_t best_k = 0, hits = 0;
#pragma unroll
  for (int k = 0; k < 6; k++) {
    const uint32_t qnx = k < 4 ? (nx >> (8 * k)) & 0xffu : (nx2 >> (8 * (k - 4))) & 0xffu, qfx = k < 4 ? (fx >> (8 * k)) & 0xffu : (fx2 >> (8 * (k - 4))) & 0xffu;
    const uint32_t qny = k < 4 ? (ny >> (8 * k)) & 0xffu : (ny2 >> (8 * (k - 4))) & 0xffu, qfy = k < 4 ? (fy >> (8 * k)) & 0xffu : (fy2 >> (8 * (k - 4))) & 0xffu;
    const uint32_t qnz = k < 4 ? (nz >> (8 * k)) & 0xffu : (nz2 >> (8 * (k - 4))) & 0xffu, qfz = k < 4 ? (fz >> (8 * k)) & 0xffu : (fz2 >> (8 * (k - 4))) & 0xffu;
    const float tnx = __builtin_fmaf((float)qnx, ax, bx), tfx = __builtin_fmaf((float)qfx, ax, bx);
    const float tny = __builtin_fmaf((float)qny, ay, by), tfy = __builtin_fmaf((float)qfy, ay, by);
    const float tnz = __builtin_fmaf((float)qnz, az, bz), tfz = __builtin_fmaf((float)qfz, az, bz);
    const float tn = fmaxf(fmaxf(fmaxf(tnx, tny), tnz), ts.tmin);
    const float tf = fminf(fminf(fminf(tfx, tfy), tfz), far_lim);
    const bool hit = (uint32_t)k < count && tn <= __builtin_fmaf(tf, kSlabSlack, 1e-30f);
    hits |= hit ? 1u << k : 0u;
    const bool nearer = hit && (uint32_t)k < n_int && tn < best_d;
    best_d = nearer ? tn : best_d;
    best_k = nearer ? (uint32_t)k : best_k;
  }
#if defined(PT_DEBUG_PID) && defined(__HIP_DEVICE_COMPILE__)
  if (ts.dbg) printf("dbg node %u: n_int %u count %u hits %x base_node %u base_leaf %u best.t %.9g\n", ts.cur, n_int, count, hits, n.base_node, n.base_leaf, ts.best.t);
#endif
  const uint32_t leaf_mask = hits >> n_int;
  ts.st.pend[(leaf_mask ? ts.st.npend : kPendLeaves6) * ts.st.lds_stride] = n.base_leaf << 6 | leaf_mask;
  ts.st.npend += leaf_mask ? 1 : 0;
  uint32_t others = hits & ((1u << n_int) - 1u);
  if (others) {
    others &= ~(1u << best_k);
    while (others) {
      const uint32_t k = (uint32_t)__builtin_ctz(others);
      others &= others - 1u;
      ts.st.push<kLdsStack6>(n.base_node + k);
    }
    ts.cur = n.base_node + best_k;
  } else {
    ts.cur = ts.st.sp == 0 ? kInvalidRef : ts.st.pop<kLdsStack6>();
  }
}

template <bool ANY, bool COUNT>
PT_HD bool trav_pending_leaf6(const DeviceScene& S, TravState& ts, TraversalCount* cnt) {
  uint32_t* top = &ts.st.pend[(ts.st.npend - 1) * ts.st.lds_stride];
  const uint32_t e = *top;
  const uint32_t mask = e & 63u, r = (uint32_t)__builtin_ctz(mask), rest = mask & (mask - 1u);
  if (rest) *top = (e & ~63u) | rest; else ts.st.npend--;
  bool finished = false;
  trav_leaf(S, ts, kLeafBit | ((e >> 6) + r), ANY, &finished, COUNT ? cnt : nullptr);
  return finished;
}

PT_HD void trav_leave(TravState& ts) {
  while (ts.cur == kExitMarker) {
    ts.co = ts.o; ts.cinv = ts.inv;
    ts.cnegx = ts.negx; ts.cnegy = ts.negy; ts.cnegz = ts.negz;
    ts.sx = ts.sy = ts.sz = 0.0f;
    ts.tri_base = 0u;
    ts.cur = ts.st.sp == 0 ? kInvalidRef : ts.st.pop();
  }
}
PT_HD void trav_resolve(const DeviceScene& S, TravState& ts) {
  for (;;) {
    if (ts.cur == kExitMarker) {
      ts.co = ts.o; ts.cinv = ts.inv;
      ts.cnegx = ts.negx; ts.cnegy = ts.negy; ts.cnegz = ts.negz;
      ts.sx = ts.sy = ts.sz = 0.0f;
      ts.tri_base = 0u;
      ts.cur = ts.st.sp == 0 ? kInvalidRef : ts.st.pop();
      continue;
    }
    if (ts.cur == kInvalidRef || !(ts.cur & kInstBit)) return;
    if (ts.st.npend > kPendLeaves - 4) return;
    const InstanceTrav it = ldg(&S.inst_trav[ts.cur & ~kInstBit]);
    const MeshTrav mt = ldg(&S.mesh_trav[it.mesh]);
    if (mt.root_ref == kInvalidRef || (mt.root_ref & kLeafBit)) {
      if (mt.root_ref != kInvalidRef) ts.st.push_leaf(kLeafBit | (it.tri_base + (mt.root_ref & ~kLeafBit)));
      ts.cur = ts.st.sp == 0 ? kInvalidRef : ts.st.pop();
      continue;
    }
    const vec3 p = ts.o - v3(it.c[0], it.c[1], it.c[2]);
    const vec3 i0 = v3(it.ic0[0], it.ic0[1], it.ic0[2]), i1 = v3(it.ic1[0], it.ic1[1], it.ic1[2]), i2 = v3(it.ic2[0], it.ic2[1], it.ic2[2]);
    ts.co = (i0 * p.x + i1 * p.y) + i2 * p.z;
    const vec3 cd = (i0 * ts.d.x + i1 * ts.d.y) + i2 * ts.d.z;
    ts.cinv = v3(1.0f / cd.x, 1.0f / cd.y, 1.0f / cd.z);
    if (!(fabsf(ts.cinv.x) <= 1e30f)) ts.cinv.x = copysignf(1e30f, cd.x);
    if (!(fabsf(ts.cinv.y) <= 1e30f)) ts.cinv.y = copysignf(1e30f, cd.y);
    if (!(fabsf(ts.cinv.z) <= 1e30f)) ts.cinv.z = copysignf(1e30f, cd.z);
    ts.cnegx = ts.cinv.x < 0.0f; ts.cnegy = ts.cinv.y < 0.0f; ts.cnegz = ts.cinv.z < 0.0f;
    const float fx = ((ts.cnegx ? mt.lo[0] : mt.hi[0]) - ts.co.x) * ts.cinv.x;
    const float fy = ((ts.cnegy ? mt.lo[1] : mt.hi[1]) - ts.co.y) * ts.cinv.y;
    const float fz = ((ts.cnegz ? mt.lo[2] : mt.hi[2]) - ts.co.z) * ts.cinv.z;
    const float t1 = fminf(fminf(fx, fy), fz);
    const float tfar = fminf(ts.best.t, fmaxf(t1, 0.0f) * 1.0001f + 1e-6f);
    const vec3 ap = v3(fabsf(p.x), fabsf(p.y), fabsf(p.z)), ad = v3(fabsf(ts.d.x), fabsf(ts.d.y), fabsf(ts.d.z));
    const vec3 a0 = v3(fabsf(i0.x), fabsf(i0.y), fabsf(i0.z)), a1 = v3(fabsf(i1.x), fabsf(i1.y), fabsf(i1.z)), a2 = v3(fabsf(i2.x), fabsf(i2.y), fabsf(i2.z));
    const vec3 mp = (a0 * ap.x + a1 * ap.y) + a2 * ap.z, md = (a0 * ad.x + a1 * ad.y) + a2 * ad.z;
    float e = 8e-6f * (fmaxf(mp.x, fmaxf(mp.y, mp.z)) + tfar * fmaxf(md.x, fmaxf(md.y, md.z))) + 1e-30f;
    if (!(e <= 1e30f)) e = 1e30f;
    ts.sx = e * fabsf(ts.cinv.x); ts.sy = e * fabsf(ts.cinv.y); ts.sz = e * fabsf(ts.cinv.z);
    ts.tri_base = it.tri_base;
    ts.st.push(kExitMarker);
    ts.cur = mt.root_ref;
  }
}

// ... 32 lines not shown
```

platinum_amd/csrc/pt_layout.h:

```cpp
#pragma once
#include "pt_math.h"

namespace pt {

PT_HD uint32_t tiles_x(uint32_t W) { return (W + 7u) / 8u; }
PT_HD uint32_t tiles_y(uint32_t H) { return (H + 7u) / 8u; }
PT_HD uint32_t tile_count(uint32_t W, uint32_t H) { return tiles_x(W) * tiles_y(H); }
PT_HD uint32_t tile_of_pixel(uint32_t x, uint32_t y, uint32_t W) { return (y >> 3) * tiles_x(W) + (x >> 3); }
PT_HD uint32_t lane_of_pixel(uint32_t x, uint32_t y) { return (y & 7u) * 8u + (x & 7u); }
struct PixelXY { uint32_t x, y; };
PT_HD PixelXY tile_pixel(uint32_t tile, uint32_t lane, uint32_t tilesX) {
  const uint32_t ty = tile / tilesX;
  return {(tile - ty * tilesX) * 8u + (lane & 7u), ty * 8u + (lane >> 3)};
}

struct Rect { uint32_t x0, y0, x1, y1; };
PT_HD bool rect_contains(const Rect& r, uint32_t x, uint32_t y) { return x >= r.x0 && x < r.x1 && y >= r.y0 && y < r.y1; }
PT_HD uint32_t rect_tiles(const Rect& r, uint32_t W, uint32_t* out, uint32_t capacity) {
  const uint32_t tilesX = tiles_x(W), tx0 = r.x0 >> 3, tx1 = (r.x1 - 1u) >> 3, ty0 = r.y0 >> 3, ty1 = (r.y1 - 1u) >> 3;
  uint32_t n = 0;
  for (uint32_t ty = ty0; ty <= ty1; ty++)
    for (uint32_t tx = tx0; tx <= tx1; tx++, n++)
      if (out && n < capacity) out[n] = ty * tilesX + tx;
  return n;
}

PT_HD uint32_t lbuf_index(uint32_t tile, uint32_t s, uint32_t nsamples, uint32_t lane) { return (tile * 64u + lane) * nsamples + s; }
PT_HD uint32_t lbuf_index_of_pixel(uint32_t p, uint32_t W, uint32_t s, uint32_t nsamples) {
  const uint32_t y = p / W, x = p - y * W;
  return lbuf_index(tile_of_pixel(x, y, W), s, nsamples, lane_of_pixel(x, y));
}
PT_HD uint32_t pixel_of_pid_1spp(uint32_t pid, uint32_t W) {
  const uint32_t lane = pid & 63u, tile = pid >> 6, tilesX = tiles_x(W);
  const uint32_t ty = tile / tilesX, tx = tile - ty * tilesX;
  return (ty * 8u + (lane >> 3)) * W + tx * 8u + (lane & 7u);
}

#ifndef PT_SEG_GROUP
#define PT_SEG_GROUP 16
#endif
constexpr uint32_t kSegGroupChunks = PT_SEG_GROUP;
PT_HD uint32_t seg_slot(uint32_t nseg, uint32_t s, uint32_t r) {
  const uint32_t k = r >> 6;
  return (((k / kSegGroupChunks) * nseg + s) * kSegGroupChunks + (k % kSegGroupChunks)) * 64u + (r & 63u);
}
PT_HD uint32_t slot_segment(uint32_t nseg, uint32_t slot) { return ((slot >> 6) / kSegGroupChunks) % nseg; }
PT_HD uint64_t seg_queue_slots(uint32_t nseg, uint32_t seg_cap) {
  const uint64_t K = seg_cap / 64u;
  return (uint64_t)nseg * ((K + kSegGroupChunks - 1) / kSegGroupChunks * kSegGroupChunks) * 64;
}
PT_HD uint32_t segment_first_tile(uint32_t nseg, uint32_t bands, uint32_t tiles_per_seg, uint32_t sg) {
  const uint32_t per_band = nseg / bands;
  return ((sg % bands) * per_band + sg / bands) * tiles_per_seg;
}
PT_HD uint32_t segment_lbuf_base(uint32_t nseg, uint32_t bands, uint32_t tiles_per_seg, uint32_t nsamples, uint32_t sg) {
  return segment_first_tile(nseg, bands, tiles_per_seg, sg) * nsamples * 64u;
}

}
```

platinum_amd/csrc/renderer.hip:

```cpp
#include <hip/hip_runtime.h>

#include <algorithm>
#include <chrono>
#include <cmath>
#include <cstdio>
#include <cstdlib>
#include <cstring>
#include <string>
#include <vector>

#include "queue_plan.h"
#include "runtime_identity.h"
#include "renderer_state.h"

using namespace pt;

namespace {
thread_local std::string g_last_error;
}
int pt_fail(int code, const std::string& msg) {
  g_last_error = msg;
  return code;
}
const std::string& pt_last_error_string() { return g_last_error; }

namespace {

struct ScopedTimer {
  pt_renderer* r;
  int cls;
  hipEvent_t start = nullptr, stop = nullptr;
  ScopedTimer(pt_renderer* r_, int cls_) : r(r_), cls(cls_) {
    if (!r->profiling) return;
    if (hipEventCreate(&start) != hipSuccess || hipEventCreate(&stop) != hipSuccess) { start = stop = nullptr; return; }
    (void)hipEventRecord(start, r->stream);
  }
  ~ScopedTimer() {
    if (!start) return;
    (void)hipEventRecord(stop, r->stream);
    r->timed.push_back({cls, start, stop});
  }
};

enum BatchMode { BATCH_RENDER, BATCH_DEBUG, BATCH_MEASURE };

int enqueue_batch(pt_renderer* r, uint32_t first, uint32_t ns, uint32_t n0, BatchMode mode, int32_t* hitlog) {
  const DeviceScene& S = r->S;
  hipStream_t s = r->stream;
  BatchCounters* ctr = r->ctr.p;
  if (hitlog && ns != 1) return fail(PT_ERR_INVALID_ARGUMENT, "the hit log is kept for one-sample batches only");
  if (ns == 0 || ns > r->samples_in_flight) return fail(PT_ERR_INVALID_ARGUMENT, "batch larger than the queues");
  PT_HIP(hipMemsetAsync(ctr, 0, sizeof(BatchCounters), s));
  const bool count = mode == BATCH_MEASURE;
  Segments seg = r->segments();
  seg.nsamples = ns;
#ifdef PT_DEBUG_PID
  if (const char* e = getenv("PTAMD_DEBUG_RAY")) {
    uint32_t x = 0, y = 0, sm = 0, b = 0;
    if (sscanf(e, "%u,%u,%u,%u", &x, &y, &sm, &b) == 4 && sm >= first && sm < first + ns) {
      const uint32_t v[2] = {lbuf_index(tile_of_pixel(x, y, S.width), sm - first, ns, lane_of_pixel(x, y)), b + 1u};
      PT_HIP(hipMemcpyAsync(&ctr->_pad[0], v, 8, hipMemcpyHostToDevice, s));
    }
  }
#endif
  const bool ad = mode == BATCH_RENDER && r->vtiles;
  const uint32_t* ad_list = ad ? r->ad_list[r->ad_cur].p : nullptr;
  const uint32_t* ad_count = ad ? r->ad_count.p + r->ad_cur : nullptr;
  {
    ScopedTimer t(r, K_RAYGEN);
    if (ad) launch_raygen_adaptive(s, r->grid, S, r->path_state(0), r->Lbuf.p, seg, first, ns, r->rect, ad_list, ad_count);
    else launch_raygen(s, r->grid, S, r->path_state(0), r->Lbuf.p, seg, ctr, first, ns);
    launch_chunk_tables(s, seg, 0, ctr, 0, 0, false);
  }
  int cur = 0;
  const bool mis = S.integrator == PT_INTEGRATOR_MIS;
  for (uint32_t b = 0; b < S.max_bounces; b++) {
    {
      ScopedTimer t(r, K_CLOSEST);
      launch_trace_closest(s, r->closest_grid, S, r->path_state(cur), r->hit.p, seg, (uint32_t)cur, ctr, b, r->spill.p, hitlog, S.width * S.height, count);
    }
    if (b == 0 && mode == BATCH_RENDER && r->aov) launch_aov(s, r->grid, r->scene_d.p, r->path_state(cur), r->hit.p, seg, r->Abuf.p);
    {
      ScopedTimer t(r, K_SHADE);
      launch_shade(s, r->shade_grid, r->scene_d.p, r->path_state(cur), r->path_state(cur ^ 1), r->hit.p, r->shadow_queue(), r->Lbuf.p, seg, (uint32_t)cur, ctr, b);
      launch_chunk_tables(s, seg, (uint32_t)(cur ^ 1), ctr, b + 1, b, mis);
    }
    if (mis) {
      ScopedTimer t(r, K_SHADOW);
      launch_trace_shadow(s, r->shadow_grid, S, r->shadow_queue(), r->Lbuf.p, seg, ctr, b, r->spill.p, count);
    }
    cur ^= 1;
  }
  if (mode == BATCH_RENDER) {
    ScopedTimer t(r, K_ACCUM);
    const uint32_t npix = S.width * S.height;
    if (r->params.flags & PT_FLAG_GMON) {
      const uint32_t buckets = r->params.gmon_buckets;
      const uint32_t total_spp = r->gmon_total_spp ? r->gmon_total_spp : r->params.spp;
      const uint32_t spb = (total_spp + buckets - 1) / buckets;
      const uint32_t f0 = n0 + r->gmon_sample_base;
      launch_accumulate_gmon(s, r->gmon_buckets_d.p, r->Lbuf.p, npix, S.width, ns, f0, spb, buckets, r->gmon_bucket_base, r->params.nonfinite_policy, ctr);
      launch_gmon(s, r->acc, r->gmon_buckets_d.p, npix, (f0 + ns - 1) / spb + 1 - r->gmon_bucket_base, r->gmon_cap);
    } else if (ad) {
      launch_accumulate_adaptive(s, r->acc, r->Lbuf.p, npix, S.width, ns, n0, r->params.nonfinite_policy, ctr, ad_list, ad_count, r->ad_tiles0,
                                 r->adaptive ? r->ad_mom.p : nullptr, r->ad_tile_n.p, r->rect);
    } else {
      launch_accumulate(s, r->acc, r->Lbuf.p, npix, S.width, ns, n0, r->params.nonfinite_policy, ctr);
    }
    if (r->aov && ad)
      launch_accumulate_aov_adaptive(s, r->aov_img.p, r->aov_img.p + npix, r->aov_img.p + 2 * (size_t)npix, r->Abuf.p, r->Lbuf.p, S.width, S.height, ns,
                                     n0, r->params.nonfinite_policy, ad_list, ad_count, r->ad_tiles0, r->rect);
    else if (r->aov)
      launch_accumulate_aov(s, r->aov_img.p, r->aov_img.p + npix, r->aov_img.p + 2 * (size_t)npix, r->Abuf.p, r->Lbuf.p, S.width, S.height, ns, n0,
                            r->params.nonfinite_policy);
  }
  if (ad && r->adaptive && r->ad_next < r->total && n0 + ns == r->ad_next) {
    {
      ScopedTimer t(r, K_ACCUM);
      PT_HIP(launch_adaptive_check(s, ad_list, ad_count, r->ad_list[r->ad_cur ^ 1].p, r->ad_count.p + (r->ad_cur ^ 1), r->ad_mom.p, S.width, r->rect,
                                   r->ad_tiles0, r->ad_next, r->adaptive_opts.threshold, r->ad_flags.p, r->ad_scratch.p, r->ad_scratch.n,
                                   r->ad_host_count));
    }
    PT_HIP(hipEventRecord(r->ad_event, s));
    r->ad_event_valid = true;
    r->ad_cur ^= 1;
    r->ad_next += r->adaptive_opts.interval;
  }
  launch_fold_counters(s, ctr, mode == BATCH_DEBUG ? r->totals.p + 1 : r->totals.p, seg, count);
  PT_HIP(hipGetLastError());
  r->last_batch_ns = ns; r->last_batch_first = first;
  return PT_OK;
}

void collect_timings(pt_renderer* r) {
  for (auto& t : r->timed) {
    float ms = 0.0f;
    if (hipEventElapsedTime(&ms, t.start, t.stop) == hipSuccess) {
      r->ms_class[t.cls] += ms;
      r->launches[t.cls]++;
    }
  }
  r->drop_timed();
}

int load_luts(pt_renderer* r, const uint8_t* b, size_t size) {
  if (size < 12 + 16 * 8 || memcmp(b, "PTLUT01\0", 8) != 0) return fail(PT_ERR_BAD_LUT, "LUT blob: bad magic (expected PTLUT01)");
  uint32_t count;
  memcpy(&count, b + 8, 4);
  if (count != 8) return fail(PT_ERR_BAD_LUT, "LUT blob: expected 8 tables (renderer_pt.hpp:154-165)");
  uint32_t hdr[32];
  memcpy(hdr, b + 12, sizeof(hdr));
  const size_t data_off = 12 + 16 * 8;
  const size_t nfloats = (size - data_off) / 4;
  const uint32_t expect[8][3] = {{128, 128, 1}, {128, 1, 1}, {32, 32, 32}, {32, 32, 1}, {32, 32, 32}, {32, 32, 32}, {32, 32, 1}, {32, 32, 1}};
  for (int i = 0; i < 8; i++) {
    const uint32_t w = hdr[4 * i], h = hdr[4 * i + 1], d = hdr[4 * i + 2], off = hdr[4 * i + 3];
    if (w != expect[i][0] || h != expect[i][1] || d != expect[i][2] || (size_t)off + (size_t)w * h * d > nfloats)
      return fail(PT_ERR_BAD_LUT, "LUT blob: unexpected table shape");
  }
  std::vector<float> data(nfloats);
  memcpy(data.data(), b + data_off, nfloats * 4);
  PT_HIP(r->lut_data.upload(data));
  Lut* ls[6] = {&r->luts.E, &r->luts.Eavg, &r->luts.EMs, &r->luts.EavgMs, &r->luts.ETransIn, &r->luts.ETransOut};
  for (int i = 0; i < 6; i++) {
    ls[i]->w = (int)hdr[4 * i]; ls[i]->h = (int)hdr[4 * i + 1]; ls[i]->depth = (int)hdr[4 * i + 2];
    ls[i]->d = r->lut_data.p + hdr[4 * i + 3];
  }
  r->lut_w_E = hdr[0];
  r->lut_w_Eavg = hdr[4];
  return PT_OK;
}

int build_halton_table(pt_renderer* r) {
  std::vector<HaltonEntry> tab;
  tab.reserve(kHaltonDims);
  for (uint32_t c = 2; (int)tab.size() < kHaltonDims; c++) {
    bool prime = true;
    for (uint32_t d = 2; d * d <= c; d++)
      if (c % d == 0) { prime = false; break; }
    if (!prime) continue;
    tab.push_back(make_halton_entry(c));
  }
  PT_HIP(r->halton.upload(tab));
  return PT_OK;
}

}

extern "C" const char* pt_last_error(void) { return g_last_error.c_str(); }

extern "C" int pt_plan_queues(uint32_t width, uint32_t height, uint32_t spp, uint32_t samples_in_flight, uint64_t free_hbm_bytes,
                              uint32_t tiles_per_seg_override, uint32_t seg_bands, pt_queue_plan* out) {
  if (!out) return fail(PT_ERR_INVALID_ARGUMENT, "pt_plan_queues: null argument");
  const char* why = "";
  const int rc = plan_queues(width, height, spp, samples_in_flight, free_hbm_bytes, tiles_per_seg_override, seg_bands, out, &why);
  return rc == PT_OK ? PT_OK : fail(rc, std::string("pt_plan_queues: ") + why);
}

std::string pt_rccl_bound_path();

extern "C" int pt_get_runtime_info(pt_runtime_info* out) {
  if (!out) return fail(PT_ERR_INVALID_ARGUMENT, "pt_get_runtime_info: null argument");
  memset(out, 0, sizeof(*out));
  const RuntimeObjects o = mapped_runtime_objects();
  auto put = [](char* dst, size_t cap, const std::string& s) { snprintf(dst, cap, "%s", s.c_str()); };
  put(out->hip_runtime_path, sizeof(out->hip_runtime_path), object_of((const void*)&hipRuntimeGetVersion));
  put(out->hsa_runtime_path, sizeof(out->hsa_runtime_path), o.hsa.empty() ? std::string() : o.hsa[0]);
  put(out->rccl_path, sizeof(out->rccl_path), pt_rccl_bound_path());
  out->hip_runtimes_mapped = (uint32_t)o.hip.size();
  out->hsa_runtimes_mapped = (uint32_t)o.hsa.size();
  out->rccl_mapped = (uint32_t)o.rccl.size();
  int v = 0;
  out->hip_runtime_version = hipRuntimeGetVersion(&v) == hipSuccess ? v : 0;
  put(out->all_mapped, sizeof(out->all_mapped), join_paths(o.hip) + " | " + join_paths(o.hsa) + " | " + join_paths(o.rccl));
  return PT_OK;
}

int dev_create(const pt_create_info* info, int device_ordinal, pt_renderer** out) {
  if (!info || !out) return fail(PT_ERR_INVALID_ARGUMENT, "pt_create: null argument");
  *out = nullptr;
  if (info->abi_version != PT_ABI_VERSION && info->abi_version != 4u) return fail(PT_ERR_INVALID_ARGUMENT, "pt_create: ABI version mismatch");
  {
    const std::string conflict = runtime_conflict();
    if (!conflict.empty()) return fail(PT_ERR_RUNTIME_CONFLICT, "pt_create: " + conflict);
  }
  int ndev = 0;
  if (hipGetDeviceCount(&ndev) != hipSuccess || ndev <= 0)
    return fail(PT_ERR_NO_DEVICE, "pt_create: no HIP device available (this library has no CPU fallback)");
  if (device_ordinal < 0 || device_ordinal >= ndev) return fail(PT_ERR_INVALID_ARGUMENT, "pt_create: bad device ordinal");
  PT_HIP(hipSetDevice(device_ordinal));
  auto* r = new pt_renderer();
  pt_default_post_options(&r->post);
  pt_default_tonemap_options(&r->tonemap);
  pt_default_denoise_options(&r->denoise);
  pt_default_despeckle_options(&r->despeckle);
  pt_default_exposure_options(&r->exposure);
  pt_default_adaptive_options(&r->adaptive_opts);
  pt_default_render_region(&r->region_opts);
  r->device = device_ordinal;
  if (const char* e = getenv("PTAMD_REFILL")) r->refill_threshold = (uint32_t)atoi(e);
  if (const char* e = getenv("PTAMD_TILES_PER_SEG")) r->tiles_per_seg_override = (uint32_t)std::max(0, atoi(e));
  if (const char* e = getenv("PTAMD_SEG_BANDS")) r->seg_bands = (uint32_t)std::max(1, std::min(64, atoi(e)));
  if (const char* e = getenv("PTAMD_TWO_LEVEL")) r->two_level_override = atoi(e) != 0 ? 1 : 0;
  if (const char* e = getenv("PTAMD_BLOCKS_PER_CU")) r->blocks_per_cu = (uint32_t)std::max(1, std::min(8, atoi(e)));
  if (const char* e = getenv("PTAMD_CLOSEST_BLOCKS_PER_CU")) r->closest_blocks_per_cu = (uint32_t)std::max(1, std::min(8, atoi(e)));
  if (const char* e = getenv("PTAMD_SHADOW_BLOCKS_PER_CU")) r->shadow_blocks_per_cu = (uint32_t)std::max(1, std::min(8, atoi(e)));
  hipDeviceProp_t prop;
  if (hipGetDeviceProperties(&prop, r->device) == hipSuccess) r->num_cu = prop.multiProcessorCount;
  int rc = PT_OK;
  do {
    if (hipStreamCreateWithFlags(&r->own_stream, hipStreamNonBlocking) != hipSuccess) { rc = fail(PT_ERR_HIP, "hipStreamCreate failed"); break; }
    r->stream = r->own_stream;
    if (hipEventCreateWithFlags(&r->batch_done, hipEventDisableTiming) != hipSuccess) { rc = fail(PT_ERR_HIP, "hipEventCreate failed"); break; }
    std::vector<uint8_t> file;
    const uint8_t* blob = (const uint8_t*)info->lut_blob;
    size_t size = (size_t)info->lut_blob_size;
    if (!blob) {
      const char* path = info->lut_path ? info->lut_path : getenv("PTAMD_LUT_PATH");
      if (!path) { rc = fail(PT_ERR_BAD_LUT, "pt_create: no LUT blob, lut_path or $PTAMD_LUT_PATH"); break; }
      FILE* f = fopen(path, "rb");
      if (!f) { rc = fail(PT_ERR_BAD_LUT, std::string("pt_create: cannot open LUT file ") + path); break; }
      fseek(f, 0, SEEK_END);
      long n = ftell(f);
      fseek(f, 0, SEEK_SET);
      file.resize((size_t)n);
      if (fread(file.data(), 1, (size_t)n, f) != (size_t)n) { fclose(f); rc = fail(PT_ERR_BAD_LUT, "pt_create: short read on LUT file"); break; }
      fclose(f);
      blob = file.data();
      size = file.size();
    }
    if ((rc = load_luts(r, blob, size)) != PT_OK) break;
    if ((rc = build_halton_table(r)) != PT_OK) break;
    if (r->ctr.alloc(1) != hipSuccess || r->totals.alloc(2) != hipSuccess) { rc = fail(PT_ERR_OUT_OF_MEMORY, "counter allocation failed"); break; }
  } while (0);
  if (rc != PT_OK) { dev_destroy(r); return rc; }
  *out = r;
  return PT_OK;
}

void dev_destroy(pt_renderer* r) {
  if (!r) return;
  (void)hipSetDevice(r->device);
  if (r->stream) (void)hipStreamSynchronize(r->stream);
  r->drop_timed();
  r->release_all();
  if (r->batch_done) (void)hipEventDestroy(r->batch_done);
  if (r->ad_event) (void)hipEventDestroy(r->ad_event);
  if (r->ad_host_count) (void)hipHostFree(r->ad_host_count);
  if (r->own_stream) (void)hipStreamDestroy(r->own_stream);
  delete r;
}

int dev_start_render(pt_renderer* r, const pt_scene_snapshot* scene, const pt_render_params* p) {
  if (!r || !scene || !p) return fail(PT_ERR_INVALID_ARGUMENT, "pt_start_render: null argument");
  if (p->width == 0 || p->height == 0 || p->spp == 0) return fail(PT_ERR_INVALID_ARGUMENT, "pt_start_render: empty size or spp");
  if (p->max_bounces < 1 || p->max_bounces > 50)
    return fail(PT_ERR_INVALID_ARGUMENT, "pt_start_render: max_bounces must be 1..50 (620 Halton dimensions, kernel.metal:5)");
  if ((uint64_t)p->width * p->height > (1ull << 28)) return fail(PT_ERR_INVALID_ARGUMENT, "pt_start_render: image too large");
  if (p->integrator != PT_INTEGRATOR_SIMPLE && p->integrator != PT_INTEGRATOR_MIS) return fail(PT_ERR_INVALID_ARGUMENT, "bad integrator");
  if (p->nonfinite_policy > PT_NONFINITE_ZERO) return fail(PT_ERR_INVALID_ARGUMENT, "bad nonfinite_policy");
  if (p->accel_structure > PT_ACCEL_TWO_LEVEL) return fail(PT_ERR_INVALID_ARGUMENT, "bad accel_structure");
  if ((p->flags & PT_FLAG_GMON) && (p->gmon_buckets < 1 || p->gmon_buckets > 32))
    return fail(PT_ERR_INVALID_ARGUMENT, "gmon_buckets must be 1..32 (gmon.metal:12 maxBuckets)");
  if (scene->instance_count && (!scene->instances || !scene->instance_materials || !scene->meshes))
    return fail(PT_ERR_INVALID_ARGUMENT, "pt_start_render: null scene arrays");
  if (r->adaptive_opts.enabled && (p->flags & PT_FLAG_GMON))
    return fail(PT_ERR_UNSUPPORTED, "pt_start_render: adaptive sampling does not support PT_FLAG_GMON (a bucket would have to be resolved per tile count)");
  if (r->region_opts.enabled) {
    const pt_render_region& g = r->region_opts;
    if (g.x1 > p->width || g.y1 > p->height)
      return fail(PT_ERR_INVALID_ARGUMENT, "pt_start_render: the render region [" + std::to_string(g.x0) + ", " + std::to_string(g.x1) + ") x [" +
                                               std::to_string(g.y0) + ", " + std::to_string(g.y1) + ") does not fit the " +
                                               std::to_string(p->width) + " x " + std::to_string(p->height) + " image");
    if (p->flags & PT_FLAG_GMON)
      return fail(PT_ERR_UNSUPPORTED, "pt_start_render: a render region does not support PT_FLAG_GMON (the GMoN kernels index the radiance buffer by image pixel)");
  }
  PT_HIP(hipSetDevice(r->device));
  if (r->stream) PT_HIP(hipStreamSynchronize(r->stream));
  r->drop_timed();
  r->free_scene();
  r->params = *p;
  r->stream = p->stream ? (hipStream_t)p->stream : r->own_stream;
  const auto t_up0 = std::chrono::steady_clock::now();
  const bool phase_log = getenv("PTAMD_START_PHASES") != nullptr;
  auto phase = [&, t_last = std::chrono::steady_clock::now()](const char* what) mutable {
    if (!phase_log) return;
    (void)hipDeviceSynchronize();
    const auto now = std::chrono::steady_clock::now();
// ... 61 lines not shown
      ~EventPair() { if (e0) (void)hipEventDestroy(e0); if (e1) (void)hipEventDestroy(e1); }
    } ev;
    PT_HIP(hipEventCreate(&ev.e0));
    PT_HIP(hipEventCreate(&ev.e1));
    PT_HIP(hipEventRecord(ev.e0, r->stream));
    uint64_t unique_tris = 0;
    for (const MeshInfo& m : hs.meshes) unique_tris += m.tri_count;
    std::vector<InstanceTrav> itrav(hs.instances.size());
    bool invertible = true;
    for (size_t i = 0; i < hs.instances.size(); i++) {
      const InstanceInfo& in = hs.instances[i];
      M3d m{};
      for (int k = 0; k < 3; k++) { m.m[0][k] = in.c0[k]; m.m[1][k] = in.c1[k]; m.m[2][k] = in.c2[k]; }
      const double det = m.m[0][0] * (m.m[1][1] * m.m[2][2] - m.m[2][1] * m.m[1][2]) - m.m[1][0] * (m.m[0][1] * m.m[2][2] - m.m[2][1] * m.m[0][2]) +
                         m.m[2][0] * (m.m[0][1] * m.m[1][2] - m.m[1][1] * m.m[0][2]);
      double scale = 0;
      for (int c = 0; c < 3; c++) for (int k = 0; k < 3; k++) scale = std::max(scale, std::fabs(m.m[c][k]));
      if (!(std::fabs(det) > 1e-12 * scale * scale * scale) || !std::isfinite(det)) { invertible = false; break; }
      const M3d inv = m3_inv(m);
      InstanceTrav& t = itrav[i];
      for (int k = 0; k < 3; k++) { t.ic0[k] = (float)inv.m[0][k]; t.ic1[k] = (float)inv.m[1][k]; t.ic2[k] = (float)inv.m[2][k]; t.c[k] = in.c3[k]; }
      t.tri_base = in.tri_global_base; t.mesh = in.mesh; t._pad[0] = t._pad[1] = 0;
    }
    {
      size_t free_b = 0, total_b = 0;
      if (hipMemGetInfo(&free_b, &total_b) != hipSuccess) free_b = 0;
      const uint64_t flat_bytes = (uint64_t)r->tri_count * 292ull;
      r->two_level = invertible && (uint64_t)r->tri_count >= 8 * unique_tris && free_b != 0 && flat_bytes > free_b / 2;
      if (r->two_level && p->accel_structure == PT_ACCEL_AUTO && r->two_level_override < 0 && !getenv("PTAMD_QUIET"))
        fprintf(stderr, "ptamd: PT_ACCEL_AUTO chose the TWO-LEVEL structure (flattening %u triangles would take %.1f GB of the %.1f GB free): 1.75x the "
                        "traversal time of one BVH, and closest hits can differ from it where fp32 Moeller-Trumbore accepts a triangle the ray passes "
                        "outside of (the seed-310601 class: ~1 pixel-sample per 1 500 scenes); PT_ACCEL_ONE_BVH / PT_ACCEL_TWO_LEVEL pin the choice\n",
                r->tri_count, (double)flat_bytes / 1e9, (double)free_b / 1e9);
    }
    if (p->accel_structure == PT_ACCEL_ONE_BVH) r->two_level = false;
    else if (p->accel_structure == PT_ACCEL_TWO_LEVEL) r->two_level = invertible;
    else if (r->two_level_override >= 0) r->two_level = invertible && r->two_level_override != 0;
    hipError_t be;
    if (r->two_level) {
      PT_HIP(r->inst_trav.upload(itrav));
      be = build_two_level(r->stream, S, hs.meshes.data(), (uint32_t)hs.meshes.size(), r->instance_count, r->tri_count,
                           (uint32_t)(kLdsStack + kSpillStack), &r->bvh_scratch, &r->bvh);
    } else {
      build_primitives(&hs, getenv("PTAMD_NO_PAIRS") == nullptr);
      PT_HIP(r->prim_tri_d.upload(hs.prim_tri));
      PT_HIP(r->mesh_prim_base_d.upload(hs.mesh_prim_base));
      PT_HIP(r->inst_prim_base_d.upload(hs.inst_prim_base));
      PrimTables prims;
      prims.prim_tri = r->prim_tri_d.p; prims.mesh_prim_base = r->mesh_prim_base_d.p; prims.inst_prim_base = r->inst_prim_base_d.p;
      prims.slot_count = hs.prim_count;
      be = build_lbvh(r->stream, S, prims, r->instance_count, (uint32_t)(kLdsStack + kSpillStack), &r->bvh_scratch, &r->bvh);
    }
    if (be != hipSuccess)
      return fail(be == hipErrorOutOfMemory ? PT_ERR_OUT_OF_MEMORY : PT_ERR_HIP, std::string("LBVH build failed: ") + hipGetErrorString(be));
    PT_HIP(hipEventRecord(ev.e1, r->stream));
    PT_HIP(hipEventSynchronize(ev.e1));
    float ms = 0;
    (void)hipEventElapsedTime(&ms, ev.e0, ev.e1);
    r->bvh_ms = ms;
    if (r->bvh.depth4 * (r->bvh.wide6 ? 5u : 3u) + (r->two_level ? 1 : 0) > (uint32_t)(kLdsStack + kSpillStack))
      return fail(PT_ERR_UNSUPPORTED, "BVH too deep for the traversal stack (degenerate geometry: thousands of coincident triangles?)");
    S.nodes = r->bvh.nodes;
    S.tris = r->bvh.tris;
    S.slot_count = r->slot_count = r->bvh.slot_count;
    S.root_ref = r->bvh.root_ref;
    S.node_count = r->bvh.node_count;
    S.two_level = r->two_level ? 1u : 0u;
    S.wide6 = r->bvh.wide6 ? 1u : 0u;
    S.inst_trav = r->inst_trav.p;
    S.mesh_trav = r->bvh.mesh_trav;
  }
  phase("acceleration structure");
  PT_HIP(r->shade_recs.alloc(std::max<size_t>(1, 2 * (size_t)r->slot_count)));
  S.shade_recs = r->shade_recs.p;
  launch_shade_records(r->stream, S, r->shade_recs.p);
  PT_HIP(r->light_recs.alloc(std::max<size_t>(1, r->lights.size())));
  PT_HIP(r->light_cdf.alloc(std::max<size_t>(1, r->lights.size())));
  S.light_recs = r->light_recs.p;
  S.light_cdf = r->light_cdf.p;
  launch_light_records(r->stream, S, r->light_recs.p, r->light_cdf.p);
  PT_HIP(r->scene_d.upload(std::vector<DeviceScene>(1, S)));

  phase("shade / light records");
  const uint64_t npix = (uint64_t)p->width * p->height;
  const bool aov = r->denoise.enabled != 0;
  if (!aov) { r->Abuf.release(); r->aov_img.release(); }
  const bool adaptive = r->adaptive_opts.enabled != 0;
  const bool region = r->region_opts.enabled != 0;
  if (!adaptive) r->release_checkpoints();
  if (!adaptive && !region) r->release_adaptive();
  const Rect rect = region ? Rect{r->region_opts.x0, r->region_opts.y0, r->region_opts.x1, r->region_opts.y1} : Rect{0u, 0u, p->width, p->height};
  {
    size_t free_b = 0, total_b = 0;
    if (hipMemGetInfo(&free_b, &total_b) != hipSuccess) free_b = 0;
    else free_b += r->queue_bytes_held();
    if (aov && free_b) {
      free_b += r->Abuf.bytes_held();
      free_b = free_b / 232 * 200;
    }
    pt_queue_plan plan{};
    const char* why = "";
    const int rc = plan_queues(p->width, p->height, p->spp, p->samples_in_flight, free_b, r->tiles_per_seg_override, r->seg_bands, &plan, &why);
    if (rc != PT_OK) return fail(rc, std::string("pt_start_render: ") + why);
    r->samples_in_flight = plan.samples_in_flight;
    r->tiles_per_seg = plan.tiles_per_seg;
    r->nseg = plan.nseg;
    r->seg_cap = plan.seg_cap;
    r->capacity = (size_t)plan.capacity;
  }
  const uint32_t sif = r->samples_in_flight;
  r->grid = (uint32_t)r->num_cu * r->blocks_per_cu;
  r->shade_grid = (uint32_t)r->num_cu * shade_blocks_per_cu();
  r->closest_grid = (uint32_t)r->num_cu * (r->two_level ? trace_blocks_per_cu_two_level() : r->closest_blocks_per_cu);
  r->shadow_grid = (uint32_t)r->num_cu * (r->two_level ? trace_blocks_per_cu_two_level() : r->shadow_blocks_per_cu);
  r->nstats = std::max(r->grid * (kBlock / 64), r->shade_grid * (shade_block_threads() / 64));
  for (int k = 0; k < 2; k++) {
    PT_HIP(r->st_rayO[k].alloc(r->capacity)); PT_HIP(r->st_rayD[k].alloc(r->capacity));
    PT_HIP(r->st_att[k].alloc(r->capacity));
  }
  PT_HIP(r->hit.alloc(r->capacity));
  PT_HIP(r->sq_o.alloc(r->capacity)); PT_HIP(r->sq_d.alloc(r->capacity)); PT_HIP(r->sq_c.alloc(r->capacity));
  PT_HIP(r->Lbuf.alloc((size_t)tile_count(p->width, p->height) * 64 * sif));
  for (int k = 0; k < 2; k++) PT_HIP(r->seg_active[k].alloc(r->nseg));
  PT_HIP(r->seg_shadow.alloc(r->nseg));
  PT_HIP(r->seg_poison.alloc(r->nseg));
  PT_HIP(r->wave_stats.alloc(r->nstats));
  for (int k = 0; k < 2; k++) PT_HIP(r->chunk_table[k].alloc(r->capacity / 64 + 8));
  PT_HIP(r->shade_order.alloc(r->nseg));
  PT_HIP(r->shade_cost.alloc((size_t)r->nseg * (r->S.max_bounces + 1u)));
  PT_HIP(hipMemsetAsync(r->shade_cost.p, 0, sizeof(uint32_t) * r->shade_cost.n, r->stream));
  PT_HIP(r->spill.alloc((size_t)std::max(r->closest_grid, r->shadow_grid) * trace_block_threads(r->two_level) * kSpillStack));
  PT_HIP(hipMemsetAsync(r->wave_stats.p, 0, sizeof(WaveStats) * r->nstats, r->stream));
  if (p->external_accumulator) {
    r->acc = (vec4*)p->external_accumulator;
  } else {
    PT_HIP(r->acc_own.alloc(npix));
    r->acc = r->acc_own.p;
  }
  if (p->flags & PT_FLAG_GMON) {
    const uint32_t own = r->gmon_own_buckets ? r->gmon_own_buckets : p->gmon_buckets;
    PT_HIP(r->gmon_buckets_d.alloc((size_t)npix * own));
    PT_HIP(hipMemsetAsync(r->gmon_buckets_d.p, 0, sizeof(vec4) * npix * own, r->stream));
  }
  PT_HIP(hipMemsetAsync(r->acc, 0, sizeof(vec4) * npix, r->stream));
  if (aov) {
    PT_HIP(r->Abuf.alloc(2 * r->Lbuf.n));
    PT_HIP(r->aov_img.alloc(3 * npix));
    PT_HIP(hipMemsetAsync(r->aov_img.p, 0, sizeof(vec4) * 3 * npix, r->stream));
  }
  if (adaptive || region) {
    const uint32_t tiles = tile_count(p->width, p->height);
    std::vector<uint32_t> first(rect_tiles(rect, p->width, nullptr, 0));
    (void)rect_tiles(rect, p->width, first.data(), (uint32_t)first.size());
    const uint32_t active = (uint32_t)first.size();
    r->ad_tiles0 = active;
    PT_HIP(r->ad_list[0].upload(first));
    PT_HIP(r->ad_list[1].upload(first));
    PT_HIP(r->ad_count.upload(std::vector<uint32_t>{active, active}));
    PT_HIP(r->ad_tile_n.alloc(tiles));
    PT_HIP(hipMemsetAsync(r->ad_tile_n.p, 0, sizeof(uint32_t) * tiles, r->stream));
    if (adaptive) {
      PT_HIP(r->ad_mom.alloc(npix));
      PT_HIP(hipMemsetAsync(r->ad_mom.p, 0, sizeof(vec2) * npix, r->stream));
      PT_HIP(r->ad_flags.alloc(active));
      PT_HIP(r->ad_scratch.alloc(std::max<size_t>(1, adaptive_scratch_bytes(active))));
      if (!r->ad_host_count) PT_HIP(hipHostMalloc((void**)&r->ad_host_count, sizeof(uint32_t), hipHostMallocDefault));
      if (!r->ad_event) PT_HIP(hipEventCreateWithFlags(&r->ad_event, hipEventDisableTiming));
      *r->ad_host_count = active;
    }
  }
  PT_HIP(hipMemsetAsync(r->totals.p, 0, sizeof(Totals), r->stream));
  PT_HIP(hipStreamSynchronize(r->stream));

  phase("queues + accumulator");
  for (int k = 0; k < K_CLASSES; k++) { r->ms_class[k] = 0; r->launches[k] = 0; }
  r->accumulated = 0;
  r->launched = 0;
  r->batches = 0;
  r->last_batch_ns = 0;
  r->batch_done_valid = false;
  r->total = p->spp;
  r->aov = aov;
  r->adaptive = adaptive;
  r->region = region;
  r->vtiles = adaptive || region;
  r->rect = rect;
  r->ad_cur = 0;
  r->ad_event_valid = false;
  r->ad_next = r->adaptive_opts.min_spp;
  r->started = true;
  r->render_start = std::chrono::steady_clock::now();
  r->timer_ms = 0;
  return PT_OK;
}

// ... 309 lines not shown
  if (!r || !out) return fail(PT_ERR_INVALID_ARGUMENT, "null argument");
  if (!r->started) return fail(PT_ERR_BAD_STATE, "pt_read_exposure_meter before pt_start_render");
  PT_HIP(hipSetDevice(r->device));
  int rc = dev_wait(r);
  if (rc != PT_OK) return rc;
  const vec4* src = acc_device ? acc_device : r->acc;
  if (!acc_device && r->aov && r->denoise.apply_to_target) {
    if ((rc = enqueue_denoise(r)) != PT_OK) return rc;
    src = r->denoised.p;
  }
  if ((rc = exposure_record(r)) != PT_OK) return rc;
  PT_HIP(launch_exposure_meter(r->stream, src, r->S.width, r->rect, r->exposure, r->exp_rec.p, false));
  PT_HIP(hipStreamSynchronize(r->stream));
  PT_HIP(hipMemcpy(out, &r->exp_rec.p->meter, sizeof(*out), hipMemcpyDeviceToHost));
  return PT_OK;
}

int dev_debug_exposure(pt_renderer* r, const float* rgba, uint32_t width, uint32_t height, const uint32_t* rect, const pt_exposure_options* options,
                       pt_exposure_meter* out, float* scaled_out) {
  if (!options || !rgba || !out) return fail(PT_ERR_INVALID_ARGUMENT, "null argument");
  if (const char* why = exposure_options_error(*options)) return fail(PT_ERR_INVALID_ARGUMENT, std::string("pt_debug_exposure: ") + why);
  if (width == 0 || height == 0 || (uint64_t)width * height > (1ull << 28)) return fail(PT_ERR_INVALID_ARGUMENT, "pt_debug_exposure: the image must hold 1..2^28 pixels");
  Rect rc{0u, 0u, width, height};
  if (rect) {
    rc = Rect{rect[0], rect[1], rect[2], rect[3]};
    if (rc.x0 >= rc.x1 || rc.y0 >= rc.y1 || rc.x1 > width || rc.y1 > height) return fail(PT_ERR_INVALID_ARGUMENT, "pt_debug_exposure: the rectangle is empty or does not fit the image");
  }
  if (!r) return fail(PT_ERR_INVALID_ARGUMENT, "pt_debug_exposure: null renderer");
  PT_HIP(hipSetDevice(r->device));
  const size_t npix = (size_t)width * height;
  DevBuf<vec4> img, scaled;
  DevBuf<ExposureRecord> rec;
  PT_HIP(img.alloc(npix)); PT_HIP(scaled.alloc(npix)); PT_HIP(rec.alloc(1));
  PT_HIP(hipMemcpyAsync(img.p, rgba, sizeof(vec4) * npix, hipMemcpyHostToDevice, r->stream));
  PT_HIP(hipMemsetAsync(rec.p, 0, sizeof(ExposureRecord), r->stream));
  PT_HIP(launch_exposure_meter(r->stream, img.p, width, rc, *options, rec.p, false));
  launch_exposure_apply(r->stream, img.p, scaled.p, (uint32_t)npix, rec.p);
  PT_HIP(hipGetLastError());
  PT_HIP(hipStreamSynchronize(r->stream));
  PT_HIP(hipMemcpy(out, &rec.p->meter, sizeof(*out), hipMemcpyDeviceToHost));
  if (scaled_out) PT_HIP(hipMemcpy(scaled_out, scaled.p, sizeof(vec4) * npix, hipMemcpyDeviceToHost));
  return PT_OK;
}

extern "C" void pt_default_adaptive_options(pt_adaptive_options* o) {
  if (!o) return;
  memset(o, 0, sizeof(*o));
  o->threshold = 0.02f;
  o->min_spp = 32;
  o->interval = 32;
}

int dev_set_adaptive_options(pt_renderer* r, const pt_adaptive_options* o) {
  if (!o) return fail(PT_ERR_INVALID_ARGUMENT, "null argument");
  if (!(o->threshold > 0.0f && o->threshold <= 3.4028234663852886e38f))
    return fail(PT_ERR_INVALID_ARGUMENT, "pt_set_adaptive_options: threshold must be finite and > 0");
  if (o->min_spp < 2) return fail(PT_ERR_INVALID_ARGUMENT, "pt_set_adaptive_options: min_spp must be >= 2");
  if (o->interval < 1) return fail(PT_ERR_INVALID_ARGUMENT, "pt_set_adaptive_options: interval must be >= 1");
  if (!r) return fail(PT_ERR_INVALID_ARGUMENT, "pt_set_adaptive_options: null renderer");
  r->adaptive_opts = *o;
  return PT_OK;
}

int dev_read_sample_counts(pt_renderer* r, uint32_t* out) {
  if (!r || !out) return fail(PT_ERR_INVALID_ARGUMENT, "null argument");
  if (!r->started) return fail(PT_ERR_BAD_STATE, "pt_read_sample_counts before pt_start_render");
  int rc = dev_wait(r);
  if (rc != PT_OK) return rc;
  const uint32_t W = r->S.width, H = r->S.height;
  if (!r->vtiles) {
    std::fill(out, out + (size_t)W * H, (uint32_t)r->launched);
    return PT_OK;
  }
  std::vector<uint32_t> tn(r->ad_tile_n.n);
  PT_HIP(hipMemcpy(tn.data(), r->ad_tile_n.p, sizeof(uint32_t) * tn.size(), hipMemcpyDeviceToHost));
  for (uint32_t y = 0; y < H; y++)
    for (uint32_t x = 0; x < W; x++) out[(size_t)y * W + x] = rect_contains(r->rect, x, y) ? tn[tile_of_pixel(x, y, W)] : 0u;
  return PT_OK;
}

extern "C" void pt_default_render_region(pt_render_region* o) {
  if (!o) return;
  memset(o, 0, sizeof(*o));
}

int dev_set_render_region(pt_renderer* r, const pt_render_region* o) {
  if (!o) return fail(PT_ERR_INVALID_ARGUMENT, "null argument");
  if (o->enabled && (o->x0 >= o->x1 || o->y0 >= o->y1))
    return fail(PT_ERR_INVALID_ARGUMENT, "pt_set_render_region: the region is empty (x0 < x1 and y0 < y1 are required)");
  if (!r) return fail(PT_ERR_INVALID_ARGUMENT, "pt_set_render_region: null renderer");
  r->region_opts = *o;
  return PT_OK;
}

extern "C" int pt_region_tiles(uint32_t width, uint32_t height, const pt_render_region* o, uint32_t* tiles_out, uint32_t capacity, uint32_t* count) {
  if (!o || !count || (capacity && !tiles_out)) return fail(PT_ERR_INVALID_ARGUMENT, "pt_region_tiles: null argument");
  if (width == 0 || height == 0) return fail(PT_ERR_INVALID_ARGUMENT, "pt_region_tiles: empty image");
  Rect rect{0u, 0u, width, height};
  if (o->enabled) {
    if (o->x0 >= o->x1 || o->y0 >= o->y1) return fail(PT_ERR_INVALID_ARGUMENT, "pt_region_tiles: the region is empty");
    if (o->x1 > width || o->y1 > height) return fail(PT_ERR_INVALID_ARGUMENT, "pt_region_tiles: the region does not fit the image");
    rect = Rect{o->x0, o->y0, o->x1, o->y1};
  }
  *count = rect_tiles(rect, width, tiles_out, capacity);
  return PT_OK;
}

int dev_postprocess_to_host(pt_renderer* r, const vec4* acc_device, uint8_t* rgba8_out) {
  PT_HIP(hipSetDevice(r->device));
  const size_t npix = (size_t)r->S.width * r->S.height;
  if (r->render_target.n != npix) PT_HIP(r->render_target.alloc(npix));
  PostConstants pc;
  pc.post = r->post;
  pc.tm = r->tonemap;
  const Mat3 odt = compute_transform(r->params.working_space, r->tonemap.output_space);
  pc.odt = PPMat3{odt.c0, odt.c1, odt.c2};
  if (r->exposure.enabled) { const int rc = enqueue_exposure(r, &acc_device); if (rc != PT_OK) return rc; }
  launch_postprocess(r->stream, acc_device, r->render_target.p, r->S.width, r->S.height, pc);
  PT_HIP(hipGetLastError());
  PT_HIP(hipStreamSynchronize(r->stream));
  PT_HIP(hipMemcpy(rgba8_out, r->render_target.p, npix * 4, hipMemcpyDeviceToHost));
  return PT_OK;
}

int dev_present(pt_renderer* r, const vec4* acc_device, void** device_rgba8_out, void** stream_out) {
  if (!r || !device_rgba8_out) return fail(PT_ERR_INVALID_ARGUMENT, "null argument");
  if (!r->started) return fail(PT_ERR_BAD_STATE, "pt_present_render_target before pt_start_render");
  PT_HIP(hipSetDevice(r->device));
  { const int rc = flush_pending(r, true); if (rc != PT_OK) return rc; }
  const size_t npix = (size_t)r->S.width * r->S.height;
  if (r->render_target.n != npix) PT_HIP(r->render_target.alloc(npix));
  PostConstants pc;
  pc.post = r->post;
  pc.tm = r->tonemap;
  const Mat3 odt = compute_transform(r->params.working_space, r->tonemap.output_space);
  pc.odt = PPMat3{odt.c0, odt.c1, odt.c2};
  const vec4* src = acc_device ? acc_device : r->acc;
  if (!acc_device && r->aov && r->denoise.apply_to_target) {
    const int rc = enqueue_denoise(r);
    if (rc != PT_OK) return rc;
    src = r->denoised.p;
  }
  if (r->exposure.enabled) { const int rc = enqueue_exposure(r, &src); if (rc != PT_OK) return rc; }
  launch_postprocess(r->stream, src, r->render_target.p, r->S.width, r->S.height, pc);
  PT_HIP(hipGetLastError());
  *device_rgba8_out = r->render_target.p;
  if (stream_out) *stream_out = (void*)r->stream;
  return PT_OK;
}

int dev_read_render_target(pt_renderer* r, uint8_t* rgba8_out) {
  if (!r || !rgba8_out) return fail(PT_ERR_INVALID_ARGUMENT, "null argument");
  if (!r->started) return fail(PT_ERR_BAD_STATE, "pt_read_render_target before pt_start_render");
  int rc = dev_wait(r);
  if (rc != PT_OK) return rc;
  if (r->aov && r->denoise.apply_to_target) {
    if ((rc = enqueue_denoise(r)) != PT_OK) return rc;
    return dev_postprocess_to_host(r, r->denoised.p, rgba8_out);
  }
  return dev_postprocess_to_host(r, r->acc, rgba8_out);
}

int dev_set_gmon_options(pt_renderer* r, const pt_gmon_options* o) {
  if (!r || !o) return fail(PT_ERR_INVALID_ARGUMENT, "null argument");
  if (!(o->cap >= 0.0f && o->cap <= 1.0f)) return fail(PT_ERR_INVALID_ARGUMENT, "gmon cap must lie in [0, 1]");
  r->gmon_cap = o->cap;
// ... 154 lines not shown
```

platinum_amd/csrc/renderer_state.h:

```cpp
#pragma once
#include <hip/hip_runtime.h>

#include <chrono>
#include <memory>
#include <string>
#include <vector>

#include "host_scene.h"
#include "adaptive.h"
#include "denoise.h"
#include "exposure.h"
#include "kernels.h"
#include "pt_bvh.h"

using namespace pt;

int pt_fail(int code, const std::string& msg);
const std::string& pt_last_error_string();
inline int fail(int code, const std::string& msg) { return pt_fail(code, msg); }

namespace {

#define PT_HIP(call)                                                                                       \
  do {                                                                                                     \
    hipError_t e_ = (call);                                                                                \
    if (e_ != hipSuccess) {                                                                                \
      char buf_[512];                                                                                      \
      snprintf(buf_, sizeof(buf_), "%s:%d: %s failed: %s", __FILE__, __LINE__, #call, hipGetErrorString(e_)); \
      return fail(e_ == hipErrorOutOfMemory ? PT_ERR_OUT_OF_MEMORY : PT_ERR_HIP, buf_);                     \
    }                                                                                                      \
  } while (0)

template <typename T>
struct DevBuf {
  T* p = nullptr;
  size_t n = 0;
  size_t cap = 0;
  hipError_t alloc(size_t count) {
    if (count <= cap) { n = count; return hipSuccess; }
    release();
    const hipError_t e = hipMalloc(reinterpret_cast<void**>(&p), sizeof(T) * count);
    if (e != hipSuccess) { p = nullptr; return e; }
    n = cap = count;
    return hipSuccess;
  }
  size_t bytes_held() const { return cap * sizeof(T); }
  hipError_t upload(const std::vector<T>& v) {
    hipError_t e = alloc(v.size());
    if (e != hipSuccess || v.empty()) return e;
    return hipMemcpy(p, v.data(), sizeof(T) * v.size(), hipMemcpyHostToDevice);
  }
  void release() {
    if (p) (void)hipFree(p);
    p = nullptr;
    n = cap = 0;
  }
  ~DevBuf() { release(); }
};

enum KernelClass { K_RAYGEN = 0, K_CLOSEST, K_SHADE, K_SHADOW, K_ACCUM, K_CLASSES };

struct TimedLaunch { int cls; hipEvent_t start, stop; };

}

struct pt_renderer {
  int device = 0;
  int num_cu = 256;
  hipStream_t own_stream = nullptr;
  hipStream_t stream = nullptr;

  DevBuf<float> lut_data;
  LutSet luts{};
  uint32_t lut_w_E = 0, lut_w_Eavg = 0;
  DevBuf<HaltonEntry> halton;

  bool started = false;
  DevBuf<pt_float3> positions;
  DevBuf<pt_vertex_data> vdata;
  DevBuf<uint32_t> indices, slots;
  DevBuf<MeshInfo> meshes;
  DevBuf<InstanceInfo> instances;
  DevBuf<pt_material_gpu> materials;
  DevBuf<pt_area_light> lights_d;
  std::vector<pt_area_light> lights;
  DevBuf<DeviceScene> scene_d;
  DevBuf<ShadeRec> shade_recs;
  DevBuf<LightRec> light_recs;
  DevBuf<float> light_cdf;
  DevBuf<uint32_t> prim_tri_d, mesh_prim_base_d, inst_prim_base_d;
  DevBuf<InstanceTrav> inst_trav;
  bool two_level = false;
  int two_level_override = -1;
  DevBuf<uint8_t> tex_data;
  DevBuf<float> tex_decode;
  DevBuf<TexInfo> textures;
  DevBuf<pt_alias_entry> env_alias_d;
  std::vector<pt_alias_entry> env_alias;
  LbvhResult bvh{};
  LbvhScratch bvh_scratch{};
  DeviceScene S{};
  pt_render_params params{};
  pt_constants constants{};
  uint32_t instance_count = 0, tri_count = 0, slot_count = 0;

  uint32_t samples_in_flight = 0;
  size_t capacity = 0;
  DevBuf<vec4> st_rayO[2], st_rayD[2], st_att[2], hit, sq_o, sq_d, sq_c, Lbuf, acc_own;
  DevBuf<uint32_t> spill, seg_active[2], seg_shadow, seg_poison;
  DevBuf<WaveStats> wave_stats;
  DevBuf<uint32_t> chunk_table[2];
  DevBuf<uint32_t> shade_order, shade_cost;
  DevBuf<vec4> gmon_buckets_d;
  float gmon_cap = 1.0f;
  pt_post_options post{};
  pt_tonemap_options tonemap{};
  DevBuf<uint32_t> render_target;
  pt_denoise_options denoise{};
  pt_despeckle_options despeckle{};
  bool aov = false;
  DevBuf<vec4> Abuf;
  DevBuf<vec4> aov_img;
  DevBuf<vec4> dn_guide, dn_aux, dn_col[2], denoised;
  pt_exposure_options exposure{};
  DevBuf<ExposureRecord> exp_rec;
  DevBuf<vec4> exp_img;
  pt_adaptive_options adaptive_opts{};
  bool adaptive = false;
  DevBuf<uint32_t> ad_list[2];
  DevBuf<uint32_t> ad_count;
  DevBuf<uint32_t> ad_tile_n;
  DevBuf<vec2> ad_mom;
  DevBuf<uint8_t> ad_flags, ad_scratch;
  uint32_t* ad_host_count = nullptr;
  hipEvent_t ad_event = nullptr;
  bool ad_event_valid = false;
  int ad_cur = 0;
  uint32_t ad_next = 0;
  pt_render_region region_opts{};
  bool region = false;
  bool vtiles = false;
  Rect rect{};
  uint32_t ad_tiles0 = 0;
  uint32_t closest_grid = 0, shadow_grid = 0, closest_blocks_per_cu = PT_CLOSEST_WAVES, shadow_blocks_per_cu = PT_SHADOW_WAVES;
  uint32_t last_batch_ns = 0, last_batch_first = 0;
  uint32_t nseg = 0, tiles_per_seg = 1, seg_bands = 4, tiles_per_seg_override = 0, nstats = 0, seg_cap = 0, blocks_per_cu = 6, shade_grid = 0, refill_threshold = 48;
  DevBuf<BatchCounters> ctr;
  DevBuf<Totals> totals;
  vec4* acc = nullptr;
  uint32_t grid = 0;

  uint32_t gmon_sample_base = 0;
  uint32_t gmon_total_spp = 0;
  uint32_t gmon_bucket_base = 0;
  uint32_t gmon_own_buckets = 0;
  struct DeviceGroup* group = nullptr;

  uint64_t accumulated = 0, total = 0, launched = 0;
  uint32_t batches = 0;
  hipEvent_t batch_done = nullptr;
  bool batch_done_valid = false;
  std::chrono::steady_clock::time_point render_start;
  uint64_t timer_ms = 0;

  bool profiling = false;
  std::vector<TimedLaunch> timed;
  double ms_class[K_CLASSES] = {0, 0, 0, 0, 0};
  uint64_t launches[K_CLASSES] = {0, 0, 0, 0, 0};
  double upload_ms = 0, bvh_ms = 0;

  PathState path_state(int k) { return PathState{st_rayO[k].p, st_rayD[k].p, st_att[k].p}; }
  ShadowQueue shadow_queue() { return ShadowQueue{sq_o.p, sq_d.p, sq_c.p}; }
  Segments segments() { return Segments{{seg_active[0].p, seg_active[1].p}, seg_shadow.p, seg_poison.p, wave_stats.p, chunk_table[0].p, chunk_table[1].p, shade_order.p, shade_cost.p, seg_cap, nseg, tiles_per_seg,  0u, seg_bands, nstats, refill_threshold}; }

  void free_scene() {
    if (bvh.nodes) (void)hipFree(bvh.nodes);
    if (bvh.tris) (void)hipFree(bvh.tris);
    if (bvh.mesh_trav) (void)hipFree(bvh.mesh_trav);
    bvh = LbvhResult{};
    acc = nullptr;
    started = false;
    aov = false;
    adaptive = false;
    region = false;
    vtiles = false;
    ad_event_valid = false;
    last_batch_ns = 0;
  }
  size_t queue_bytes_held() const {
    size_t b = hit.bytes_held() + sq_o.bytes_held() + sq_d.bytes_held() + sq_c.bytes_held() + Lbuf.bytes_held() + chunk_table[0].bytes_held() + chunk_table[1].bytes_held();
    for (int k = 0; k < 2; k++) b += st_rayO[k].bytes_held() + st_rayD[k].bytes_held() + st_att[k].bytes_held();
    return b;
  }
  void release_all() {
    free_scene();
    positions.release(); vdata.release(); indices.release(); slots.release(); meshes.release(); instances.release();
    materials.release(); lights_d.release(); tex_data.release(); tex_decode.release(); textures.release(); env_alias_d.release(); scene_d.release(); shade_recs.release(); light_recs.release(); light_cdf.release();
    inst_trav.release(); prim_tri_d.release(); mesh_prim_base_d.release(); inst_prim_base_d.release();
    bvh_scratch.release();
    for (int k = 0; k < 2; k++) { st_rayO[k].release(); st_rayD[k].release(); st_att[k].release(); }
    seg_active[0].release(); seg_active[1].release(); seg_shadow.release(); seg_poison.release(); wave_stats.release(); chunk_table[0].release(); chunk_table[1].release(); shade_order.release(); shade_cost.release(); gmon_buckets_d.release(); render_target.release();
    hit.release(); sq_o.release(); sq_d.release(); sq_c.release(); Lbuf.release(); acc_own.release(); spill.release();
    Abuf.release(); aov_img.release(); dn_guide.release(); dn_aux.release(); dn_col[0].release(); dn_col[1].release(); denoised.release();
    exp_rec.release(); exp_img.release();
    release_adaptive();
  }
  void release_adaptive() {
    release_checkpoints();
    ad_list[0].release(); ad_list[1].release(); ad_count.release(); ad_tile_n.release();
  }
  void release_checkpoints() { ad_mom.release(); ad_flags.release(); ad_scratch.release(); }
  void drop_timed() {
    for (auto& t : timed) { (void)hipEventDestroy(t.start); (void)hipEventDestroy(t.stop); }
    timed.clear();
  }
};


int dev_create(const pt_create_info* info, int device_ordinal, pt_renderer** out);
void dev_destroy(pt_renderer* r);
int dev_start_render(pt_renderer* r, const pt_scene_snapshot* scene, const pt_render_params* p);
int dev_render_step(pt_renderer* r, uint32_t max_spp);
int dev_wait(pt_renderer* r);
int dev_status(const pt_renderer* r);
int dev_progress(const pt_renderer* r, uint64_t* accumulated, uint64_t* total);
uint64_t dev_render_time_ms(const pt_renderer* r);
int dev_read_accumulator(pt_renderer* r, float* rgba_out);
int dev_set_post_options(pt_renderer* r, const pt_post_options* o);
int dev_set_tonemap_options(pt_renderer* r, const pt_tonemap_options* o);
int dev_read_render_target(pt_renderer* r, uint8_t* rgba8_out);
int dev_postprocess_to_host(pt_renderer* r, const vec4* acc_device, uint8_t* rgba8_out);
int dev_present(pt_renderer* r, const vec4* acc_device, void** device_rgba8_out, void** stream_out);
int dev_set_gmon_options(pt_renderer* r, const pt_gmon_options* o);
int dev_read_gmon_bucket(pt_renderer* r, uint32_t bucket, float* rgba_out);
void* dev_accumulator_device_ptr(pt_renderer* r);
int dev_get_constants(const pt_renderer* r, pt_constants* out);
int dev_get_lights(const pt_renderer* r, pt_area_light* out, uint32_t capacity, uint32_t* count);
int dev_get_env_alias(const pt_renderer* r, pt_alias_entry* out, uint64_t capacity, uint64_t* count);
int dev_trace_primary(pt_renderer* r, uint32_t sample_idx, pt_hit_record* out);
int dev_debug_sample(pt_renderer* r, uint32_t sample_idx, float* radiance_out, int32_t* hits_out);
int dev_measure_traversal(pt_renderer* r, uint32_t sample_idx);
int dev_set_profiling(pt_renderer* r, int enabled);
int dev_get_stats(pt_renderer* r, pt_stats* out);
int dev_set_denoise_options(pt_renderer* r, const pt_denoise_options* o);
int dev_read_aov(pt_renderer* r, uint32_t aov, float* rgba_out);
int dev_read_denoised(pt_renderer* r, float* rgba_out);
int dev_set_despeckle_options(pt_renderer* r, const pt_despeckle_options* o);
int dev_set_exposure_options(pt_renderer* r, const pt_exposure_options* o);
int dev_reset_exposure(pt_renderer* r);
int dev_read_exposure_meter(pt_renderer* r, const vec4* acc_device, pt_exposure_meter* out);
int dev_debug_exposure(pt_renderer* r, const float* rgba, uint32_t width, uint32_t height, const uint32_t* rect, const pt_exposure_options* options,
                       pt_exposure_meter* out, float* scaled_out);
int dev_set_adaptive_options(pt_renderer* r, const pt_adaptive_options* o);
int dev_read_sample_counts(pt_renderer* r, uint32_t* out);
int dev_set_render_region(pt_renderer* r, const pt_render_region* o);
```

platinum_amd/renderer.py:

```python
import ctypes as C

import numpy as np

from . import abi, scenes


def make_params(width, height, spp, max_bounces, flags=abi.FLAG_MULTISCATTER_GGX, integrator=abi.INTEGRATOR_MIS,
                working_space=scenes.BT2020, gmon_buckets=1, first_sample=0, samples_in_flight=0,
                external_accumulator=None, stream=None, nonfinite_policy=abi.NONFINITE_PROPAGATE, accel_structure=abi.ACCEL_AUTO):
    p = abi.RenderParams()
    p.accel_structure = accel_structure
    p.width, p.height, p.spp, p.gmon_buckets = width, height, spp, gmon_buckets
    p.flags, p.integrator = flags, integrator
    p.working_space = scenes.colorspace(working_space)
    p.max_bounces, p.first_sample, p.samples_in_flight = max_bounces, first_sample, samples_in_flight
    p.nonfinite_policy = nonfinite_policy
    p.external_accumulator = external_accumulator
    p.stream = stream
    return p


class Renderer:
    Integrator_Simple, Integrator_MIS = abi.INTEGRATOR_SIMPLE, abi.INTEGRATOR_MIS
    Status_Blocked, Status_Ready, Status_Busy, Status_Done = 0, 1, 4, 8
# ... 181 lines not shown
        o = self.adaptiveOptions() if o is None else o
        for k, v in fields.items():
            setattr(o, k, v)
        abi.check(self._lib, self._lib.pt_set_adaptive_options(self._h, C.byref(o)))
        self._adaptive = o

    def readbackSampleCounts(self):
        w, h = self.size
        out = np.empty((h, w), dtype=np.uint32)
        abi.check(self._lib, self._lib.pt_read_sample_counts(self._h, out.ctypes.data))
        return out

    def renderRegion(self):
        if getattr(self, "_region", None) is None:
            self._region = abi.RenderRegion()
            self._lib.pt_default_render_region(C.byref(self._region))
        o = abi.RenderRegion()
        C.memmove(C.byref(o), C.byref(self._region), C.sizeof(o))
        return o

    def setRenderRegion(self, x0, y0, x1, y1):
        o = abi.RenderRegion(1, x0, y0, x1, y1)
        abi.check(self._lib, self._lib.pt_set_render_region(self._h, C.byref(o)))
        self._region = o

    def clearRenderRegion(self):
        o = abi.RenderRegion()
        self._lib.pt_default_render_region(C.byref(o))
        abi.check(self._lib, self._lib.pt_set_render_region(self._h, C.byref(o)))
        self._region = o

    def setGmonOptions(self, cap=1.0):
        o = abi.GmonOptions(cap)
        abi.check(self._lib, self._lib.pt_set_gmon_options(self._h, C.byref(o)))

    def readGmonBucket(self, bucket):
        w, h = self.size
        out = np.empty((h, w, 4), dtype=np.float32)
        abi.check(self._lib, self._lib.pt_read_gmon_bucket(self._h, bucket, out.ctypes.data))
        return out

    def accumulatorDevicePtr(self):
        return self._lib.pt_accumulator_device_ptr(self._h)

    def constants(self):
        c = abi.Constants()
        abi.check(self._lib, self._lib.pt_get_constants(self._h, C.byref(c)))
        return c

    def lights(self):
        n = C.c_uint32()
        abi.check(self._lib, self._lib.pt_get_lights(self._h, None, 0, C.byref(n)))
        arr = (abi.AreaLight * max(1, n.value))()
        abi.check(self._lib, self._lib.pt_get_lights(self._h, arr, n.value, C.byref(n)))
        return list(arr)[: n.value]

    def envAlias(self):
        n = C.c_uint64()
        abi.check(self._lib, self._lib.pt_get_env_alias(self._h, None, 0, C.byref(n)))
        arr = np.zeros(n.value, dtype=abi.ALIAS_DTYPE)
        if n.value:
            abi.check(self._lib, self._lib.pt_get_env_alias(self._h, arr.ctypes.data, n.value, C.byref(n)))
        return arr

    def tracePrimary(self, sample_idx=0):
        w, h = self.size
        out = np.zeros(w * h, dtype=[("t", "f4"), ("u", "f4"), ("v", "f4"), ("instance", "i4"), ("primitive", "i4")])
        abi.check(self._lib, self._lib.pt_trace_primary(self._h, sample_idx, out.ctypes.data))
        return out.reshape(h, w)

    def debugSample(self, sample_idx):
        w, h = self.size
        B = self._params.max_bounces
        rad = np.zeros((h, w, 4), dtype=np.float32)
        hits = np.zeros((B, h, w, 2), dtype=np.int32)
        abi.check(self._lib, self._lib.pt_debug_sample(self._h, sample_idx, rad.ctypes.data, hits.ctypes.data))
        return rad, hits

    def stats(self):
        s = abi.Stats()
        abi.check(self._lib, self._lib.pt_get_stats(self._h, C.byref(s)))
        return s

    def setProfiling(self, enabled):
        abi.check(self._lib, self._lib.pt_set_profiling(self._h, int(enabled)))

    def measureTraversal(self, sample_idx=0):
        abi.check(self._lib, self._lib.pt_measure_traversal(self._h, sample_idx))
```

Baseline: 9522 Msamples/s.

## Precompute per-pixel camera leaf lists for primary-ray traversal

Adds a one-time kernel at start-up that walks the wide BVH with a per-tile camera cone. For each pixel it stores a distance-sorted list of leaf nodes its pixel cone touches, with overflow pixels flagged to fall back to normal traversal. On bounce 0, primary rays then test only the listed leaves with early exit by distance instead of walking the full BVH from the root. Flagged pixels run through a filtered version of the ordinary closest-hit kernel. The cost is extra device memory, a build pass at start, a second launch when any pixel overflows, and the feature switches off for depth of field, adaptive sampling, render regions and two-level acceleration structures.

```diff
diff --git a/include/ptamd.h b/include/ptamd.h
--- a/include/ptamd.h
+++ b/include/ptamd.h
@@ -325,6 +325,19 @@
 void pt_default_render_region(pt_render_region* o);
 int pt_set_render_region(pt_renderer* r, const pt_render_region* o);
 int pt_region_tiles(uint32_t width, uint32_t height, const pt_render_region* o, uint32_t* tiles_out, uint32_t capacity, uint32_t* count);
+
+#define PT_CAMLIST_HIST_BINS 65
+typedef struct pt_camera_list_stats {
+  uint32_t built;
+  uint32_t capacity;
+  uint64_t pixels_listed;
+  uint64_t pixels_walk;
+  uint64_t entries;
+  double build_ms;
+  uint32_t length_histogram[PT_CAMLIST_HIST_BINS];
+  uint32_t _pad;
+} pt_camera_list_stats;
+int pt_get_camera_list_stats(pt_renderer* r, pt_camera_list_stats* out);
 
 const char* pt_last_error(void);
 
diff --git a/platinum_amd/abi.py b/platinum_amd/abi.py
--- a/platinum_amd/abi.py
+++ b/platinum_amd/abi.py
@@ -187,6 +187,11 @@
 
 class RenderRegion(C.Structure):
     _fields_ = [("enabled", C.c_uint32), ("x0", C.c_uint32), ("y0", C.c_uint32), ("x1", C.c_uint32), ("y1", C.c_uint32)]
+
+
+class CameraListStats(C.Structure):
+    _fields_ = [("built", C.c_uint32), ("capacity", C.c_uint32), ("pixels_listed", C.c_uint64), ("pixels_walk", C.c_uint64),
+                ("entries", C.c_uint64), ("build_ms", C.c_double), ("length_histogram", C.c_uint32 * 65), ("_pad", C.c_uint32)]
 
 
 class HitRecord(C.Structure):
@@ -261,6 +266,7 @@
     ("pt_default_render_region", None, [C.POINTER(RenderRegion)]),
     ("pt_set_render_region", C.c_int, [C.c_void_p, C.POINTER(RenderRegion)]),
     ("pt_region_tiles", C.c_int, [C.c_uint32, C.c_uint32, C.POINTER(RenderRegion), C.c_void_p, C.c_uint32, C.POINTER(C.c_uint32)]),
+    ("pt_get_camera_list_stats", C.c_int, [C.c_void_p, C.POINTER(CameraListStats)]),
     ("pt_last_error", C.c_char_p, []),
     ("pt_get_constants", C.c_int, [C.c_void_p, C.POINTER(Constants)]),
     ("pt_get_lights", C.c_int, [C.c_void_p, C.c_void_p, C.c_uint32, C.POINTER(C.c_uint32)]),
diff --git a/platinum_amd/csrc/camera_lists.h b/platinum_amd/csrc/camera_lists.h
--- /dev/null
+++ b/platinum_amd/csrc/camera_lists.h
@@ -0,0 +1,18 @@
+#pragma once
+#include <hip/hip_runtime.h>
+
+#include "pt_camlist.h"
+
+namespace pt {
+
+struct CamListCounters {
+  unsigned long long listed;
+  unsigned long long walk;
+  unsigned long long entries;
+  uint32_t hist[kCamHistBins];
+  uint32_t _pad;
+};
+
+void launch_camera_lists(hipStream_t s, const DeviceScene& S, CamListEntry* entries, uint32_t* count, uint32_t cap, CamListCounters* counters);
+
+}
diff --git a/platinum_amd/csrc/camera_lists.hip b/platinum_amd/csrc/camera_lists.hip
--- /dev/null
+++ b/platinum_amd/csrc/camera_lists.hip
@@ -0,0 +1,74 @@
+#include <hip/hip_runtime.h>
+
+#include "camera_lists.h"
+#include "kernels.h"
+
+namespace pt {
+
+__global__ void __launch_bounds__(kBlock) k_camera_lists(DeviceScene S, CamListEntry* __restrict__ entries, uint32_t* __restrict__ count, uint32_t cap,
+                                                         uint32_t tilesX, uint32_t tiles, CamListCounters* __restrict__ out) {
+  __shared__ uint32_t lds_stack[kBlock / 64][kCamStack];
+  const uint32_t lane = wave_lane(), w = threadIdx.x >> 6;
+  const uint32_t tile = blockIdx.x * (kBlock / 64) + w;
+  if (tile >= tiles) return;
+  uint32_t* stack = lds_stack[w];
+  const uint32_t ty = tile / tilesX, tx = tile - ty * tilesX;
+  const PixelXY q = tile_pixel(tile, lane, tilesX);
+  const bool valid = q.x < S.width && q.y < S.height;
+  const CamCone tile_cone = cam_tile_cone(S.camera, tx, ty);
+  const CamCone pix_cone = cam_pixel_cone(S.camera, q.x, q.y);
+  const BvhNode6* __restrict__ nodes = reinterpret_cast<const BvhNode6*>(S.nodes);
+  CamListEntry* list = entries + (size_t)(tile * 64u + lane) * cap;
+  uint32_t len = 0;
+  bool overflow = false;
+  uint32_t sp = 0, cur = S.root_ref;
+  while (cur != kInvalidRef) {
+    const BvhNode6 n = nodes[cur];
+    const uint32_t n_int = n.counts & 7u, n_all = n_int + ((n.counts >> 3) & 7u);
+    const bool touched = lane < n_all && !cam_box_outside(tile_cone, cam_child_box(n, lane < 6u ? lane : 0u));
+    const uint32_t mask = (uint32_t)__ballot(touched) & 63u;
+    const uint32_t leaves = mask >> n_int;
+    uint32_t inner = mask & ((1u << n_int) - 1u);
+    if (leaves && valid) {
+      float dist = 0.0f;
+      const uint32_t mine = cam_node_leaves(n, pix_cone, leaves, &dist);
+      if (mine) {
+        if (len < cap) cam_list_insert(list, len, cur << 6 | mine, dist);
+        len++;
+      }
+    }
+    while (inner) {
+      const uint32_t k = (uint32_t)__builtin_ctz(inner);
+      inner &= inner - 1u;
+      if (sp < kCamStack) stack[sp++] = n.base_node + k; else overflow = true;
+    }
+    cur = sp ? stack[--sp] : kInvalidRef;
+    cur = (uint32_t)__builtin_amdgcn_readfirstlane((int)cur);
+  }
+  const bool fits = !overflow && len <= cap;
+  count[tile * 64u + lane] = !valid ? 0u : fits ? len : kCamWalk;
+  const unsigned long long m_listed = __ballot(valid && fits), m_walk = __ballot(valid && !fits);
+  uint32_t total = valid && fits ? len : 0u;
+  for (int off = 32; off > 0; off >>= 1) total += __shfl_xor(total, off, 64);
+  if (lane == 0) {
+    if (m_listed) atomicAdd(&out->listed, (unsigned long long)__popcll(m_listed));
+    if (m_walk) atomicAdd(&out->walk, (unsigned long long)__popcll(m_walk));
+    if (total) atomicAdd(&out->entries, (unsigned long long)total);
+  }
+  const uint32_t bin = len < kCamHistBins - 1u ? len : kCamHistBins - 1u;
+  unsigned long long left = __ballot(valid);
+  while (left) {
+    const uint32_t b = (uint32_t)__builtin_amdgcn_readlane((int)bin, __builtin_ctzll(left));
+    const unsigned long long same = __ballot(valid && bin == b);
+    if (lane == 0) atomicAdd(&out->hist[b], (uint32_t)__popcll(same));
+    left &= ~same;
+  }
+}
+
+void launch_camera_lists(hipStream_t s, const DeviceScene& S, CamListEntry* entries, uint32_t* count, uint32_t cap, CamListCounters* counters) {
+  const uint32_t tiles = tile_count(S.width, S.height);
+  hipLaunchKernelGGL(k_camera_lists, dim3((tiles + kBlock / 64 - 1) / (kBlock / 64)), dim3(kBlock), 0, s, S, entries, count, cap, tiles_x(S.width), tiles,
+                     counters);
+}
+
+}
diff --git a/platinum_amd/csrc/kernels.h b/platinum_amd/csrc/kernels.h
--- a/platinum_amd/csrc/kernels.h
+++ b/platinum_amd/csrc/kernels.h
@@ -1,6 +1,7 @@
 #pragma once
 #include <hip/hip_runtime.h>
 
+#include "pt_camlist.h"
 #include "pt_device.h"
 #include "pt_layout.h"
 #include "pt_post.h"
@@ -42,6 +43,9 @@
 uint32_t trace_blocks_per_cu_two_level();
 void launch_trace_closest(hipStream_t s, uint32_t grid, const DeviceScene& S, PathState st, vec4* hit, Segments seg, uint32_t cur,
                           BatchCounters* ctr, uint32_t bounce, uint32_t* spill, int32_t* hitlog, uint32_t log_stride, bool count);
+void launch_trace_camera(hipStream_t s, uint32_t grid, uint32_t grid_unlisted, const DeviceScene& S, PathState st, vec4* hit, Segments seg,
+                         BatchCounters* ctr, uint32_t* spill, const CameraLists& cl, bool any_unlisted);
+uint32_t camera_blocks_per_cu();
 uint32_t shade_block_threads();
 uint32_t shade_blocks_per_cu();
 void launch_shade(hipStream_t s, uint32_t grid, const DeviceScene* S_device, PathState sin, PathState sout, const vec4* hit,
diff --git a/platinum_amd/csrc/kernels.hip b/platinum_amd/csrc/kernels.hip
--- a/platinum_amd/csrc/kernels.hip
+++ b/platinum_amd/csrc/kernels.hip
@@ -1,6 +1,7 @@
 #include <hip/hip_runtime.h>
 
 #include "kernels.h"
+#include "pt_camlist.h"
 #include "pt_denoise.h"
 #include "pt_post.h"
 #include "pt_shade.h"
@@ -312,10 +313,10 @@
   return lds_nodes;
 }
 
-template <bool COUNT, bool TWO, bool W6 = false>
-__global__ void __launch_bounds__(TWO ? kTraceBlock2 : kBlock, TWO ? PT_TWO_BLOCKS_PER_CU : PT_CLOSEST_WAVES)
-k_trace_closest(DeviceScene S, PathState st, vec4* __restrict__ hit, Segments seg, uint32_t cur, BatchCounters* __restrict__ ctr, uint32_t bounce,
-                uint32_t* __restrict__ spill, int32_t* __restrict__ hitlog, uint32_t log_stride) {
+template <bool COUNT, bool TWO, bool W6, bool UNLISTED>
+__device__ __forceinline__ void trace_closest_body(const DeviceScene& S, PathState st, vec4* __restrict__ hit, const Segments& seg, uint32_t cur,
+                                                   BatchCounters* __restrict__ ctr, uint32_t bounce, uint32_t* __restrict__ cursor,
+                                                   uint32_t* __restrict__ spill, int32_t* __restrict__ hitlog, uint32_t log_stride, const CameraLists& cl) {
   PT_TAIL_BEGIN
   constexpr uint32_t kTB = TWO ? kTraceBlock2 : kBlock;
   __shared__ uint32_t lds_stack[(W6 ? kLdsStack6 : kLdsStack) + 1][kTB];
@@ -324,7 +325,7 @@
   const BvhNode* lds_nodes = TWO && kLdsNodes ? stage_nodes(S, lds_nodes_buf) : nullptr;
   const uint32_t lane = wave_lane();
   ChunkClaims src;
-  src.init(seg.table_closest, ctr->chunks_closest[bounce], &ctr->work_closest[bounce], seg, lane);
+  src.init(seg.table_closest, ctr->chunks_closest[bounce], cursor, seg, lane);
   TraversalStack stack;
   stack.lds = &lds_stack[0][threadIdx.x];
   stack.pend = &lds_pend[0][threadIdx.x];
@@ -365,7 +366,9 @@
       ts.dbg = ctr->_pad[1] == bounce + 1u && segment_lbuf_base(seg, slot_segment(seg.nseg, ray)) + (f2u(d4.w) >> kMetaPidShift) == ctr->_pad[0];
       if (ts.dbg) printf("dbg ray slot %u lane %u wave %u o %.9g %.9g %.9g d %.9g %.9g %.9g\n", ray, lane, wave_index(), o4.x, o4.y, o4.z, d4.x, d4.y, d4.z);
 #endif
-      if (trav_init(S, ts, v3(o4.x, o4.y, o4.z), v3(d4.x, d4.y, d4.z), 1e-3f, kInf, ir, stack, false, COUNT ? &tc : nullptr)) finish();
+      if (UNLISTED && cl.count[pixel_slot_of_pid(segment_lbuf_base(seg, slot_segment(seg.nseg, ray)) + (f2u(d4.w) >> kMetaPidShift), seg.nsamples)] != kCamWalk)
+        ray = kInvalidRef;
+      else if (trav_init(S, ts, v3(o4.x, o4.y, o4.z), v3(d4.x, d4.y, d4.z), 1e-3f, kInf, ir, stack, false, COUNT ? &tc : nullptr)) finish();
     }
     PT_TAIL_T(tail_setup)
     if (__ballot(ray != kInvalidRef) == 0) {
@@ -386,6 +389,68 @@
     }
   }
   PT_TAIL_END(0)
+}
+
+template <bool COUNT, bool TWO, bool W6 = false>
+__global__ void __launch_bounds__(TWO ? kTraceBlock2 : kBlock, TWO ? PT_TWO_BLOCKS_PER_CU : PT_CLOSEST_WAVES)
+k_trace_closest(DeviceScene S, PathState st, vec4* __restrict__ hit, Segments seg, uint32_t cur, BatchCounters* __restrict__ ctr, uint32_t bounce,
+                uint32_t* __restrict__ spill, int32_t* __restrict__ hitlog, uint32_t log_stride) {
+  trace_closest_body<COUNT, TWO, W6, false>(S, st, hit, seg, cur, ctr, bounce, &ctr->work_closest[bounce], spill, hitlog, log_stride, CameraLists{});
+}
+
+#ifndef PT_CAMERA_WAVES
+#define PT_CAMERA_WAVES 6
+#endif
+__global__ void __launch_bounds__(kBlock, PT_CAMERA_WAVES)
+k_trace_camera(DeviceScene S, PathState st, vec4* __restrict__ hit, Segments seg, BatchCounters* __restrict__ ctr, CameraLists cl) {
+  const uint32_t lane = wave_lane();
+  ChunkClaims src;
+  src.init(seg.table_closest, ctr->chunks_closest[0], &ctr->work_closest[0], seg, lane);
+  const BvhNode6* __restrict__ nodes = reinterpret_cast<const BvhNode6*>(S.nodes);
+  for (;;) {
+    const uint32_t ray = src.take(true);
+    if (__ballot(ray != kInvalidRef) == 0) break;
+    if (ray != kInvalidRef) {
+      const vec4 o4 = st.rayO[ray];
+      const vec4 d4 = st.rayD[ray];
+      const uint32_t q = pixel_slot_of_pid(segment_lbuf_base(seg, slot_segment(seg.nseg, ray)) + (f2u(d4.w) >> kMetaPidShift), seg.nsamples);
+      const uint32_t len = cl.count[q];
+      if (len != kCamWalk) {
+        float ir = 0.0f;
+        if (S.has_alpha) ir = Halton{halton_table(S.halton), f2u(st.att[ray].w), f2u(d4.w) & kMetaDimMask}.sample1d();
+        TravState ts;
+        (void)trav_init(S, ts, v3(o4.x, o4.y, o4.z), v3(d4.x, d4.y, d4.z), 1e-3f, kInf, ir, TraversalStack{}, false, nullptr);
+        const CamListEntry* __restrict__ list = cl.entries + (size_t)q * cl.cap;
+        const CamListEntry none{0u, kInf};
+        CamListEntry e = len ? list[0] : none;
+        uint32_t i = 0, m = 0, base_leaf = 0;
+        for (;;) {
+          if (m == 0u) {
+            if (i >= len || e.dist > ts.best.t * kCamCullSlack) break;
+            const BvhNode6 n = nodes[e.ref >> 6];
+            m = node6_leaf_hits(n, ts, ts.best.t * kCamCullSlack) & e.ref & 63u;
+            base_leaf = n.base_leaf;
+            i++;
+            e = i < len ? list[i] : none;
+          } else {
+            const uint32_t r = (uint32_t)__builtin_ctz(m);
+            m &= m - 1u;
+            bool fin = false;
+            trav_leaf(S, ts, kLeafBit | (base_leaf + r), false, &fin, nullptr);
+          }
+        }
+        const RayHit& h = ts.best;
+        hit[ray] = vec4{h.t, h.u, h.v, u2f(h.tri == kInvalidRef ? kInvalidRef : (h.tri | ((h.gid & 3u) << 28)))};
+      }
+    }
+  }
+}
+
+constexpr uint32_t kUnlistedCursor = 63;
+__global__ void __launch_bounds__(kBlock, PT_CLOSEST_WAVES)
+k_trace_closest_unlisted(DeviceScene S, PathState st, vec4* __restrict__ hit, Segments seg, BatchCounters* __restrict__ ctr, uint32_t* __restrict__ spill,
+                         CameraLists cl) {
+  trace_closest_body<false, false, true, true>(S, st, hit, seg, 0u, ctr, 0u, &ctr->work_closest[kUnlistedCursor], spill, nullptr, 0u, cl);
 }
 
 #ifndef PT_SHADE_WAVES
@@ -929,6 +994,12 @@
   else
     hipLaunchKernelGGL((k_trace_closest<false, false>), dim3(grid), dim3(kBlock), 0, s, S, st, hit, seg, cur, ctr, bounce, spill, hitlog, log_stride);
 }
+void launch_trace_camera(hipStream_t s, uint32_t grid, uint32_t grid_unlisted, const DeviceScene& S, PathState st, vec4* hit, Segments seg,
+                         BatchCounters* ctr, uint32_t* spill, const CameraLists& cl, bool any_unlisted) {
+  hipLaunchKernelGGL(k_trace_camera, dim3(grid), dim3(kBlock), 0, s, S, st, hit, seg, ctr, cl);
+  if (any_unlisted) hipLaunchKernelGGL(k_trace_closest_unlisted, dim3(grid_unlisted), dim3(kBlock), 0, s, S, st, hit, seg, ctr, spill, cl);
+}
+uint32_t camera_blocks_per_cu() { return PT_CAMERA_WAVES; }
 uint32_t shade_block_threads() { return kShadeBlock; }
 uint32_t shade_blocks_per_cu() { return (PT_SHADE_WAVES * 4 * 64) / PT_SHADE_BLOCK; }
 void launch_shade(hipStream_t s, uint32_t grid, const DeviceScene* S, PathState sin, PathState sout, const vec4* hit,
diff --git a/platinum_amd/csrc/multi_device.hip b/platinum_amd/csrc/multi_device.hip
--- a/platinum_amd/csrc/multi_device.hip
+++ b/platinum_amd/csrc/multi_device.hip
@@ -726,6 +726,15 @@
   return PT_OK;
 }
 
+int pt_get_camera_list_stats(pt_renderer* r, pt_camera_list_stats* out) {
+  if (!is_group(r)) return dev_get_camera_list_stats(r, out);
+  if (!out) return fail(PT_ERR_INVALID_ARGUMENT, "null argument");
+  DeviceGroup* grp = r->group;
+  pt_renderer* m = grp->started ? first_started(grp) : nullptr;
+  if (!m) return fail(PT_ERR_BAD_STATE, "pt_get_camera_list_stats before pt_start_render");
+  return dev_get_camera_list_stats(m, out);
+}
+
 int pt_read_sample_counts(pt_renderer* r, uint32_t* out) {
   if (!is_group(r)) return dev_read_sample_counts(r, out);
   if (!out) return fail(PT_ERR_INVALID_ARGUMENT, "null argument");
diff --git a/platinum_amd/csrc/pt_bvh.h b/platinum_amd/csrc/pt_bvh.h
--- a/platinum_amd/csrc/pt_bvh.h
+++ b/platinum_amd/csrc/pt_bvh.h
@@ -377,10 +377,7 @@
   return n;
 }
 
-template <bool COUNT>
-PT_HD void trav_node6(const BvhNode* __restrict__ nodes, TravState& ts, TraversalCount* cnt) {
-  const BvhNode6 n = reinterpret_cast<const BvhNode6*>(nodes)[ts.cur];
-  if (COUNT) cnt->nodes++;
+PT_HD uint32_t node6_slabs(const BvhNode6& n, const TravState& ts, float far_lim, uint32_t* best_k_out) {
   const float ax = node_scale(n.exp[0]) * ts.inv.x, ay = node_scale(n.exp[1]) * ts.inv.y, az = node_scale(n.exp[2]) * ts.inv.z;
   const float bx = (n.origin[0] - ts.o.x) * ts.inv.x, by = (n.origin[1] - ts.o.y) * ts.inv.y, bz = (n.origin[2] - ts.o.z) * ts.inv.z;
   const uint32_t nx = ts.negx ? n.q[0][1] : n.q[0][0], fx = ts.negx ? n.q[0][0] : n.q[0][1];
@@ -390,7 +387,6 @@
   const uint32_t ny2 = ts.negy ? n.q[1][2] >> 16 : n.q[1][2], fy2 = ts.negy ? n.q[1][2] : n.q[1][2] >> 16;
   const uint32_t nz2 = ts.negz ? n.q[2][2] >> 16 : n.q[2][2], fz2 = ts.negz ? n.q[2][2] : n.q[2][2] >> 16;
   const uint32_t n_int = n.counts & 7u, count = n_int + ((n.counts >> 3) & 7u);
-  const float far_lim = ts.best.t * kCullSlack;
   float best_d = kInf;
   uint32_t best_k = 0, hits = 0;
 #pragma unroll
@@ -409,8 +405,23 @@
     best_d = nearer ? tn : best_d;
     best_k = nearer ? (uint32_t)k : best_k;
   }
+  *best_k_out = best_k;
+  return hits;
+}
+PT_HD uint32_t node6_leaf_hits(const BvhNode6& n, const TravState& ts, float far_lim) {
+  uint32_t best_k;
+  return node6_slabs(n, ts, far_lim, &best_k) >> (n.counts & 7u);
+}
+
+template <bool COUNT>
+PT_HD void trav_node6(const BvhNode* __restrict__ nodes, TravState& ts, TraversalCount* cnt) {
+  const BvhNode6 n = reinterpret_cast<const BvhNode6*>(nodes)[ts.cur];
+  if (COUNT) cnt->nodes++;
+  uint32_t best_k;
+  const uint32_t hits = node6_slabs(n, ts, ts.best.t * kCullSlack, &best_k);
+  const uint32_t n_int = n.counts & 7u;
 #if defined(PT_DEBUG_PID) && defined(__HIP_DEVICE_COMPILE__)
-  if (ts.dbg) printf("dbg node %u: n_int %u count %u hits %x base_node %u base_leaf %u best.t %.9g\n", ts.cur, n_int, count, hits, n.base_node, n.base_leaf, ts.best.t);
+  if (ts.dbg) printf("dbg node %u: n_int %u count %u hits %x base_node %u base_leaf %u best.t %.9g\n", ts.cur, n_int, n_int + ((n.counts >> 3) & 7u), hits, n.base_node, n.base_leaf, ts.best.t);
 #endif
   const uint32_t leaf_mask = hits >> n_int;
   ts.st.pend[(leaf_mask ? ts.st.npend : kPendLeaves6) * ts.st.lds_stride] = n.base_leaf << 6 | leaf_mask;
diff --git a/platinum_amd/csrc/pt_camlist.h b/platinum_amd/csrc/pt_camlist.h
--- /dev/null
+++ b/platinum_amd/csrc/pt_camlist.h
@@ -0,0 +1,120 @@
+#pragma once
+#include "pt_bvh.h"
+
+namespace pt {
+
+constexpr double kCamConeMargin = 1.0 / 16.0;
+constexpr uint32_t kCamWalk = 0xffffffffu;
+constexpr uint32_t kCamListCapacity = 128;
+constexpr uint32_t kCamListMaxCapacity = 128;
+constexpr float kCamCullSlack = 1.01f;
+constexpr uint32_t kCamStack = 160;
+constexpr uint32_t kCamHistBins = PT_CAMLIST_HIST_BINS;
+
+struct CamListEntry { uint32_t ref; float dist; };
+static_assert(sizeof(CamListEntry) == 8, "CamListEntry");
+
+struct CameraLists { const CamListEntry* entries; const uint32_t* count; uint32_t cap; };
+
+struct CamCone { double apex[3]; double n[4][3]; };
+struct DBox { double lo[3], hi[3]; };
+
+PT_HD CamCone cam_cone(const pt_camera_data& cam, double x0, double y0, double x1, double y1) {
+  CamCone c;
+  const double p[3] = {cam.position.x, cam.position.y, cam.position.z}, tl[3] = {cam.topLeft.x, cam.topLeft.y, cam.topLeft.z};
+  const double du[3] = {cam.pixelDeltaU.x, cam.pixelDeltaU.y, cam.pixelDeltaU.z}, dv[3] = {cam.pixelDeltaV.x, cam.pixelDeltaV.y, cam.pixelDeltaV.z};
+  const double xs[4] = {x0, x1, x1, x0}, ys[4] = {y0, y0, y1, y1};
+  double d[4][3], mid[3] = {0.0, 0.0, 0.0};
+  for (int i = 0; i < 4; i++)
+    for (int a = 0; a < 3; a++) { d[i][a] = (tl[a] + xs[i] * du[a] + ys[i] * dv[a]) - p[a]; mid[a] += d[i][a]; }
+  for (int a = 0; a < 3; a++) c.apex[a] = p[a];
+  for (int i = 0; i < 4; i++) {
+    const double* u = d[i]; const double* v = d[(i + 1) & 3];
+    double n[3] = {u[1] * v[2] - u[2] * v[1], u[2] * v[0] - u[0] * v[2], u[0] * v[1] - u[1] * v[0]};
+    const double s = n[0] * mid[0] + n[1] * mid[1] + n[2] * mid[2];
+    for (int a = 0; a < 3; a++) c.n[i][a] = s < 0.0 ? -n[a] : n[a];
+  }
+  return c;
+}
+PT_HD CamCone cam_pixel_cone(const pt_camera_data& cam, uint32_t px, uint32_t py) {
+  return cam_cone(cam, (double)px - kCamConeMargin, (double)py - kCamConeMargin, (double)px + 1.0 + kCamConeMargin, (double)py + 1.0 + kCamConeMargin);
+}
+PT_HD CamCone cam_tile_cone(const pt_camera_data& cam, uint32_t tx, uint32_t ty) {
+  return cam_cone(cam, (double)(tx * 8u) - kCamConeMargin, (double)(ty * 8u) - kCamConeMargin, (double)(tx * 8u) + 8.0 + kCamConeMargin,
+                  (double)(ty * 8u) + 8.0 + kCamConeMargin);
+}
+
+PT_HD bool cam_box_outside(const CamCone& c, const DBox& b) {
+  for (int i = 0; i < 4; i++) {
+    double s = 0.0;
+    for (int a = 0; a < 3; a++) {
+      const double l = c.n[i][a] * (b.lo[a] - c.apex[a]), h = c.n[i][a] * (b.hi[a] - c.apex[a]);
+      s += l > h ? l : h;
+    }
+    if (s < 0.0) return true;
+  }
+  return false;
+}
+
+PT_HD DBox cam_child_box(const BvhNode6& n, uint32_t k) {
+  DBox b;
+  for (int a = 0; a < 3; a++) {
+    const uint32_t ql = k < 4u ? (n.q[a][0] >> (8u * k)) & 0xffu : (n.q[a][2] >> (8u * (k - 4u))) & 0xffu;
+    const uint32_t qh = k < 4u ? (n.q[a][1] >> (8u * k)) & 0xffu : (n.q[a][2] >> (8u * (k - 4u) + 16u)) & 0xffu;
+    const float s = node_scale(n.exp[a]);
+    b.lo[a] = (double)(n.origin[a] + (float)ql * s);
+    b.hi[a] = (double)(n.origin[a] + (float)qh * s);
+  }
+  return b;
+}
+PT_HD void cam_box_union(DBox& u, const DBox& b) {
+  for (int a = 0; a < 3; a++) { u.lo[a] = b.lo[a] < u.lo[a] ? b.lo[a] : u.lo[a]; u.hi[a] = b.hi[a] > u.hi[a] ? b.hi[a] : u.hi[a]; }
+}
+PT_HD float cam_entry_dist(const CamCone& c, const DBox& b) {
+  double s = 0.0;
+  for (int a = 0; a < 3; a++) {
+    const double d = c.apex[a] < b.lo[a] ? b.lo[a] - c.apex[a] : (c.apex[a] > b.hi[a] ? c.apex[a] - b.hi[a] : 0.0);
+    s += d * d;
+  }
+  return (float)(sqrt(s) * (1.0 - 1e-6));
+}
+
+PT_HD uint32_t cam_node_leaves(const BvhNode6& n, const CamCone& c, uint32_t candidates, float* dist) {
+  const uint32_t n_int = n.counts & 7u;
+  uint32_t mask = 0;
+  DBox u;
+  for (int a = 0; a < 3; a++) { u.lo[a] = 1e300; u.hi[a] = -1e300; }
+  for (uint32_t r = 0; r < 6u; r++) {
+    if (!((candidates >> r) & 1u)) continue;
+    const DBox b = cam_child_box(n, n_int + r);
+    if (cam_box_outside(c, b)) continue;
+    mask |= 1u << r;
+    cam_box_union(u, b);
+  }
+  if (mask) *dist = cam_entry_dist(c, u);
+  return mask;
+}
+
+PT_HD void cam_list_insert(CamListEntry* list, uint32_t len, uint32_t ref, float dist) {
+  uint32_t j = len;
+  while (j > 0u && list[j - 1u].dist > dist) { list[j] = list[j - 1u]; j--; }
+  list[j] = CamListEntry{ref, dist};
+}
+
+PT_HD void cam_trace_list(const DeviceScene& S, TravState& ts, const CamListEntry* list, uint32_t len) {
+  const BvhNode6* nodes = reinterpret_cast<const BvhNode6*>(S.nodes);
+  for (uint32_t i = 0; i < len; i++) {
+    const CamListEntry e = list[i];
+    if (e.dist > ts.best.t * kCamCullSlack) break;
+    const BvhNode6 n = nodes[e.ref >> 6];
+    uint32_t m = node6_leaf_hits(n, ts, ts.best.t * kCamCullSlack) & e.ref & 63u;
+    while (m) {
+      const uint32_t r = (uint32_t)__builtin_ctz(m);
+      m &= m - 1u;
+      bool fin = false;
+      trav_leaf(S, ts, kLeafBit | (n.base_leaf + r), false, &fin, nullptr);
+    }
+  }
+}
+
+}
diff --git a/platinum_amd/csrc/pt_layout.h b/platinum_amd/csrc/pt_layout.h
--- a/platinum_amd/csrc/pt_layout.h
+++ b/platinum_amd/csrc/pt_layout.h
@@ -35,6 +35,8 @@
   const uint32_t ty = tile / tilesX, tx = tile - ty * tilesX;
   return (ty * 8u + (lane >> 3)) * W + tx * 8u + (lane & 7u);
 }
+PT_HD uint32_t pixel_slot_of_pid(uint32_t pid, uint32_t nsamples) { return nsamples == 1u ? pid : pid / nsamples; }
+PT_HD uint32_t pixel_of_pid(uint32_t pid, uint32_t nsamples, uint32_t W) { return pixel_of_pid_1spp(pixel_slot_of_pid(pid, nsamples), W); }
 
 #ifndef PT_SEG_GROUP
 #define PT_SEG_GROUP 16
diff --git a/platinum_amd/csrc/renderer.hip b/platinum_amd/csrc/renderer.hip
--- a/platinum_amd/csrc/renderer.hip
+++ b/platinum_amd/csrc/renderer.hip
@@ -77,7 +77,11 @@
   for (uint32_t b = 0; b < S.max_bounces; b++) {
     {
       ScopedTimer t(r, K_CLOSEST);
-      launch_trace_closest(s, r->closest_grid, S, r->path_state(cur), r->hit.p, seg, (uint32_t)cur, ctr, b, r->spill.p, hitlog, S.width * S.height, count);
+      if (b == 0 && mode == BATCH_RENDER && r->cam_lists)
+        launch_trace_camera(s, r->camera_grid, r->closest_grid, S, r->path_state(cur), r->hit.p, seg, ctr, r->spill.p,
+                            CameraLists{r->cam_entries.p, r->cam_count.p, r->cam_cap}, r->cam_stats.pixels_walk != 0);
+      else
+        launch_trace_closest(s, r->closest_grid, S, r->path_state(cur), r->hit.p, seg, (uint32_t)cur, ctr, b, r->spill.p, hitlog, S.width * S.height, count);
     }
     if (b == 0 && mode == BATCH_RENDER && r->aov) launch_aov(s, r->grid, r->scene_d.p, r->path_state(cur), r->hit.p, seg, r->Abuf.p);
     {
@@ -244,6 +248,8 @@
   if (const char* e = getenv("PTAMD_TWO_LEVEL")) r->two_level_override = atoi(e) != 0 ? 1 : 0;
   if (const char* e = getenv("PTAMD_BLOCKS_PER_CU")) r->blocks_per_cu = (uint32_t)std::max(1, std::min(8, atoi(e)));
   if (const char* e = getenv("PTAMD_CLOSEST_BLOCKS_PER_CU")) r->closest_blocks_per_cu = (uint32_t)std::max(1, std::min(8, atoi(e)));
+  if (const char* e = getenv("PTAMD_NO_CAMERA_LISTS")) r->no_camera_lists = atoi(e) != 0;
+  if (const char* e = getenv("PTAMD_TEST_CAMLIST_CAP")) r->cam_cap_override = (uint32_t)std::max(1, std::min((int)kCamListMaxCapacity, atoi(e)));
   if (const char* e = getenv("PTAMD_SHADOW_BLOCKS_PER_CU")) r->shadow_blocks_per_cu = (uint32_t)std::max(1, std::min(8, atoi(e)));
   hipDeviceProp_t prop;
   if (hipGetDeviceProperties(&prop, r->device) == hipSuccess) r->num_cu = prop.multiProcessorCount;
@@ -471,6 +477,52 @@
   PT_HIP(r->scene_d.upload(std::vector<DeviceScene>(1, S)));
 
   phase("shade / light records");
+
+  {
+    r->cam_stats = pt_camera_list_stats{};
+    const bool want = !r->no_camera_lists && !r->two_level && r->bvh.wide6 && S.root_ref != kInvalidRef && !(S.root_ref & kLeafBit) &&
+                      !(S.camera.apertureRadius > 0.0f) && !r->adaptive_opts.enabled && !r->region_opts.enabled;
+    const uint32_t cap = r->cam_cap_override ? r->cam_cap_override : kCamListCapacity;
+    const size_t slots = (size_t)tile_count(p->width, p->height) * 64;
+    const size_t bytes = slots * ((size_t)cap * sizeof(CamListEntry) + sizeof(uint32_t));
+    size_t free_b = 0, total_b = 0;
+    if (hipMemGetInfo(&free_b, &total_b) != hipSuccess) free_b = 0;
+    free_b += r->cam_entries.bytes_held() + r->cam_count.bytes_held();
+    if (want && bytes <= free_b / 16) {
+      PT_HIP(r->cam_entries.alloc(slots * cap));
+      PT_HIP(r->cam_count.alloc(slots));
+      PT_HIP(r->cam_counters.alloc(1));
+      PT_HIP(hipMemsetAsync(r->cam_counters.p, 0, sizeof(CamListCounters), r->stream));
+      struct EventPair {
+        hipEvent_t e0 = nullptr, e1 = nullptr;
+        ~EventPair() { if (e0) (void)hipEventDestroy(e0); if (e1) (void)hipEventDestroy(e1); }
+      } ev;
+      PT_HIP(hipEventCreate(&ev.e0));
+      PT_HIP(hipEventCreate(&ev.e1));
+      PT_HIP(hipEventRecord(ev.e0, r->stream));
+      launch_camera_lists(r->stream, S, r->cam_entries.p, r->cam_count.p, cap, r->cam_counters.p);
+      PT_HIP(hipEventRecord(ev.e1, r->stream));
+      PT_HIP(hipEventSynchronize(ev.e1));
+      PT_HIP(hipGetLastError());
+      float ms = 0;
+      (void)hipEventElapsedTime(&ms, ev.e0, ev.e1);
+      CamListCounters c{};
+      PT_HIP(hipMemcpy(&c, r->cam_counters.p, sizeof(c), hipMemcpyDeviceToHost));
+      r->cam_cap = cap;
+      r->cam_lists = true;
+      r->cam_stats.built = 1u;
+      r->cam_stats.capacity = cap;
+      r->cam_stats.pixels_listed = c.listed;
+      r->cam_stats.pixels_walk = c.walk;
+      r->cam_stats.entries = c.entries;
+      r->cam_stats.build_ms = ms;
+      for (uint32_t k = 0; k < kCamHistBins; k++) r->cam_stats.length_histogram[k] = c.hist[k];
+    } else {
+      r->release_camera_lists();
+    }
+  }
+  phase("camera lists");
+
   const uint64_t npix = (uint64_t)p->width * p->height;
   const bool aov = r->denoise.enabled != 0;
   if (!aov) { r->Abuf.release(); r->aov_img.release(); }
@@ -483,6 +535,7 @@
     size_t free_b = 0, total_b = 0;
     if (hipMemGetInfo(&free_b, &total_b) != hipSuccess) free_b = 0;
     else free_b += r->queue_bytes_held();
+    if (free_b) free_b += r->cam_entries.bytes_held() + r->cam_count.bytes_held();
     if (aov && free_b) {
       free_b += r->Abuf.bytes_held();
       free_b = free_b / 232 * 200;
@@ -500,6 +553,7 @@
   const uint32_t sif = r->samples_in_flight;
   r->grid = (uint32_t)r->num_cu * r->blocks_per_cu;
   r->shade_grid = (uint32_t)r->num_cu * shade_blocks_per_cu();
+  r->camera_grid = (uint32_t)r->num_cu * camera_blocks_per_cu();
   r->closest_grid = (uint32_t)r->num_cu * (r->two_level ? trace_blocks_per_cu_two_level() : r->closest_blocks_per_cu);
   r->shadow_grid = (uint32_t)r->num_cu * (r->two_level ? trace_blocks_per_cu_two_level() : r->shadow_blocks_per_cu);
   r->nstats = std::max(r->grid * (kBlock / 64), r->shade_grid * (shade_block_threads() / 64));
@@ -975,6 +1029,13 @@
 extern "C" void pt_default_render_region(pt_render_region* o) {
   if (!o) return;
   memset(o, 0, sizeof(*o));
+}
+
+int dev_get_camera_list_stats(pt_renderer* r, pt_camera_list_stats* out) {
+  if (!r || !out) return fail(PT_ERR_INVALID_ARGUMENT, "null argument");
+  if (!r->started) return fail(PT_ERR_BAD_STATE, "pt_get_camera_list_stats before pt_start_render");
+  *out = r->cam_stats;
+  return PT_OK;
 }
 
 int dev_set_render_region(pt_renderer* r, const pt_render_region* o) {
diff --git a/platinum_amd/csrc/renderer_state.h b/platinum_amd/csrc/renderer_state.h
--- a/platinum_amd/csrc/renderer_state.h
+++ b/platinum_amd/csrc/renderer_state.h
@@ -8,6 +8,7 @@
 
 #include "host_scene.h"
 #include "adaptive.h"
+#include "camera_lists.h"
 #include "denoise.h"
 #include "exposure.h"
 #include "kernels.h"
@@ -142,6 +143,14 @@
   bool vtiles = false;
   Rect rect{};
   uint32_t ad_tiles0 = 0;
+  DevBuf<CamListEntry> cam_entries;
+  DevBuf<uint32_t> cam_count;
+  DevBuf<CamListCounters> cam_counters;
+  bool cam_lists = false;
+  bool no_camera_lists = false;
+  uint32_t cam_cap = 0, cam_cap_override = 0;
+  pt_camera_list_stats cam_stats{};
+  uint32_t camera_grid = 0;
   uint32_t closest_grid = 0, shadow_grid = 0, closest_blocks_per_cu = PT_CLOSEST_WAVES, shadow_blocks_per_cu = PT_SHADOW_WAVES;
   uint32_t last_batch_ns = 0, last_batch_first = 0;
   uint32_t nseg = 0, tiles_per_seg = 1, seg_bands = 4, tiles_per_seg_override = 0, nstats = 0, seg_cap = 0, blocks_per_cu = 6, shade_grid = 0, refill_threshold = 48;
@@ -181,6 +190,7 @@
     acc = nullptr;
     started = false;
     aov = false;
+    cam_lists = false;
     adaptive = false;
     region = false;
     vtiles = false;
@@ -203,8 +213,10 @@
     hit.release(); sq_o.release(); sq_d.release(); sq_c.release(); Lbuf.release(); acc_own.release(); spill.release();
     Abuf.release(); aov_img.release(); dn_guide.release(); dn_aux.release(); dn_col[0].release(); dn_col[1].release(); denoised.release();
     exp_rec.release(); exp_img.release();
+    release_camera_lists(); cam_counters.release();
     release_adaptive();
   }
+  void release_camera_lists() { cam_entries.release(); cam_count.release(); cam_lists = false; }
   void release_adaptive() {
     release_checkpoints();
     ad_list[0].release(); ad_list[1].release(); ad_count.release(); ad_tile_n.release();
@@ -254,3 +266,4 @@
 int dev_set_adaptive_options(pt_renderer* r, const pt_adaptive_options* o);
 int dev_read_sample_counts(pt_renderer* r, uint32_t* out);
 int dev_set_render_region(pt_renderer* r, const pt_render_region* o);
+int dev_get_camera_list_stats(pt_renderer* r, pt_camera_list_stats* out);
diff --git a/platinum_amd/renderer.py b/platinum_amd/renderer.py
--- a/platinum_amd/renderer.py
+++ b/platinum_amd/renderer.py
@@ -287,6 +287,11 @@
         abi.check(self._lib, self._lib.pt_get_stats(self._h, C.byref(s)))
         return s
 
+    def cameraListStats(self):
+        s = abi.CameraListStats()
+        abi.check(self._lib, self._lib.pt_get_camera_list_stats(self._h, C.byref(s)))
+        return s
+
     def setProfiling(self, enabled):
         abi.check(self._lib, self._lib.pt_set_profiling(self._h, int(enabled)))
 
```

After: 10150 Msamples/s (median of 6 runs). 6.5% higher.
